# samanklesaria/traffic-env

Measured on AMD Instinct MI355X. Metric: vehicle_updates_per_sec, higher is better.
Workload: dtype f32; 1 GPU; cfg2: 4096 envs/GPU, 16x16 grid, L=400m, CAPACITY=66 (64 cars/road max), 48-car prefill, 1 spawn/entry road/8 ticks, 20-tick light cycle; settle_ticks=100, envs_per_gpu=4096, grid=16x16, cars_per_road_max=64, car_layout=transposed, parallelism=env-sharded x1

## Files before the change

### include/tfx.h

```cpp
#ifndef TFX_H
#define TFX_H

#include <stdint.h>

#ifdef __cplusplus
extern "C" {
#endif

#define TFX_ABI_VERSION 13
#define TFX_KP 2
#define TFX_MAX_ARCH 64

enum {
  TFX_OK = 0,
  TFX_EINVAL = -1,
  TFX_ESTATE = -2,
  TFX_EDEVICE = -3,
  TFX_ENOMEM = -4
};

enum {
  TFX_ACTION_BUFFER = 0,
  TFX_ACTION_BROADCAST = 1,
  TFX_ACTION_CYCLE = 2,
  TFX_ACTION_GREEDY = 3
};

enum {
  TFX_SPAWN_NONE = 0,
  TFX_SPAWN_COUNTS = 1,
  TFX_SPAWN_PERIODIC = 2
};

typedef struct tfx_config {
  int32_t m, n;
  int32_t capacity;
  int32_t n_envs;
  int32_t planes;
  float length;
  float rate;
  float car_v, car_l, car_a, car_delta, car_v0, car_b, car_T, car_s0;
  int32_t yellow_ticks;
  float thresh;
  float detect_dist;
  float overflow_penalty;
  float eps;
  int32_t learn_switch;
  int32_t validate;
  uint32_t entry_spec;
  int32_t env_id_offset;
  int32_t layout;
  int32_t n_archetypes;
  float arch[TFX_MAX_ARCH][8];
} tfx_config;

typedef struct tfx_buffers {
  float *xv;
  float *w;
  int32_t *leading;
  int32_t *lastcar;
  int32_t *obs;
  float *rewards;
  int32_t *waiting;
  uint8_t *passed_dst;
  int32_t *done_tick;
  float *trip_times;
  int32_t *n_trips;
  int32_t trip_cap;
} tfx_buffers;

typedef struct tfx_handle_s *tfx_handle;

int tfx_abi_version(void);
const char *tfx_last_error(void);

int tfx_create(const tfx_config *cfg, tfx_handle *out);
int tfx_destroy(tfx_handle h);
int tfx_dims(tfx_handle h, int32_t *I, int32_t *r, int32_t *R, int32_t *n_entry);
int tfx_tables(tfx_handle h, int32_t *dest, int32_t *phases, int32_t *nexts, int32_t *entrypoints);
int tfx_bind_buffers(tfx_handle h, const tfx_buffers *b);

int tfx_reset(tfx_handle h, const int32_t *phase_init, void *stream);
int tfx_reset_envs(tfx_handle h, const int32_t *phase_init, const uint8_t *mask, void *stream);
int tfx_refresh(tfx_handle h, void *stream);

int tfx_set_actions(tfx_handle h, int32_t mode, const int32_t *dev, int32_t period, int32_t per_tick);
int tfx_set_spawns(tfx_handle h, int32_t mode, const int32_t *dev, int32_t period, int32_t per_tick);
int tfx_set_poisson(tfx_handle h, double cars_per_tick, uint64_t seed, const uint32_t *cdf, int32_t n_cdf);
int tfx_set_regular(tfx_handle h, int32_t every, int32_t burst, uint64_t seed);
int tfx_set_spawn_archetypes(tfx_handle h, const uint8_t *dev, int32_t per_road, int32_t per_tick);

typedef struct tfx_demand {
  int32_t n_profiles, n_segments, seg_ticks, tick_offset, n_cdf;
  const uint32_t *count_cdf, *road_cdf;
  const int32_t *profile_of_env;
  uint64_t seed;
} tfx_demand;
int tfx_set_demand(tfx_handle h, const tfx_demand *dm);
int tfx_demand_counts(tfx_handle h, int32_t tick0, int32_t n_ticks, int32_t *out, void *stream);

int tfx_set_demand_mixed(tfx_handle h, const tfx_demand *dm, const uint32_t *row_cdf, int32_t n_rows);
int tfx_demand_rows(tfx_handle h, int32_t tick0, int32_t n_ticks, int32_t *counts, uint8_t *rows, void *stream);
int tfx_demand_rows_per_road(tfx_handle h, int32_t *per_road);

int tfx_step(tfx_handle h, int32_t n_ticks, void *stream);
int tfx_move_cars(tfx_handle h, void *stream);
int tfx_advance_finished_cars(tfx_handle h, void *stream);

int tfx_agent_step(tfx_handle h, int32_t n_ticks, int32_t remi, float *aobs, float *areward,
                   uint8_t *adone, void *stream);

typedef struct tfx_episode_buffers {
  float *ep_return;
  int32_t *ep_len;
  float *final_return;
  int32_t *final_len;
  uint8_t *truncated;
  int32_t *ep_index;
} tfx_episode_buffers;
int tfx_set_episodes(tfx_handle h, int32_t enabled, int32_t max_decisions, uint64_t seed, const tfx_episode_buffers *b);

int tfx_set_episode_pool(tfx_handle h, tfx_handle pool);

int tfx_remi(tfx_handle h, void *stream);
int tfx_cars_on_roads(tfx_handle h, int32_t *out, void *stream);
int tfx_done(tfx_handle h, uint8_t *out, int32_t since_tick, void *stream);

int tfx_get_tick(tfx_handle h, int32_t *tick);
int tfx_set_tick(tfx_handle h, int32_t tick);
int tfx_vehicle_updates(tfx_handle h, uint64_t *out, void *stream);
int tfx_reset_counters(tfx_handle h, void *stream);
int tfx_profile(tfx_handle h, int32_t max_ticks);
int tfx_profile_read(tfx_handle h, double *move_ms, double *advance_ms, int32_t *n_ticks);
int tfx_xv_pairs(tfx_handle h, int64_t *pairs);
int tfx_export_ring(tfx_handle h, float *ring_xv, float *ring_w, uint8_t *ring_a, void *stream);
int tfx_import_ring(tfx_handle h, const float *ring_xv, const float *ring_w, const uint8_t *ring_a, void *stream);

int tfx_fastdiv_status(tfx_handle h, int32_t *enabled, uint64_t *mismatches);
int tfx_launch_info(tfx_handle h, int32_t *grid, int32_t *block, int32_t *waves_per_road);
int tfx_fused_ticks(tfx_handle h, int64_t *ticks, int32_t *capable);
int tfx_pair_ticks(tfx_handle h, int64_t *ticks);
int tfx_tail_ticks(tfx_handle h, int64_t *ticks);
int tfx_slow_pairs(tfx_handle h, uint64_t *pairs, void *stream);
int tfx_split_ticks(tfx_handle h, int64_t *ticks);
const char *tfx_step_kernel(tfx_handle h);

int tfx_debug_fail_after(tfx_handle h, int32_t n_launches);

enum { TFX_CLONE_STREAM = 1, TFX_CLONE_EPISODE = 2 };
int tfx_clone_envs(tfx_handle dst, tfx_handle src, const int32_t *src_of_env, int32_t flags, void *stream);
int tfx_clone_skipped(tfx_handle h, uint64_t *skipped, void *stream);
typedef struct tfx_measure_buffers {
  int32_t *n_cars;
  int32_t *n_halted;
  int32_t *queue;
  float *speed_sum;
} tfx_measure_buffers;
enum { TFX_MEASURE_ACCUMULATE = 1 };
int tfx_road_measures(tfx_handle h, float halt_speed, float x_from, const tfx_measure_buffers *out, int32_t flags,
                      void *stream);
int tfx_measure_launch(tfx_handle h, int32_t *grid, int32_t *waves);
#define TFX_MAX_CELLS 32
typedef struct tfx_cell_buffers {
  int32_t *n_cars;
  float *speed_sum;
} tfx_cell_buffers;
enum { TFX_CELLS_ACCUMULATE = 1 };
int tfx_road_cells(tfx_handle h, const float *edges, int32_t n_cells, const tfx_cell_buffers *out, int32_t flags,
                   void *stream);
int tfx_cells_launch(tfx_handle h, int32_t n_cells, int32_t *grid, int32_t *waves);
#define TFX_FRAME_PX_MIN 8
#define TFX_FRAME_PX_MAX 256
enum { TFX_FRAMES_ROADS_ONLY = 1 };
int tfx_frame_size(tfx_handle h, int32_t px, int32_t *height, int32_t *width);
int tfx_frames(tfx_handle h, const int32_t *env_ids, int32_t n_frames, int32_t px, uint8_t *out, int32_t flags,
               void *stream);
int tfx_frames_launch(tfx_handle h, int32_t n_frames, int32_t px, int32_t *grid, int32_t *waves);
typedef struct tfx_age_buffers {
  int32_t *n_cars;
  int64_t *age_sum;
  int32_t *age_max;
} tfx_age_buffers;
enum { TFX_TRAVEL_ACCUMULATE = 1 };
int tfx_car_ages(tfx_handle h, const tfx_age_buffers *out, int32_t flags, void *stream);
int tfx_ages_launch(tfx_handle h, int32_t *grid, int32_t *waves);
typedef struct tfx_trip_stat_buffers {
  int32_t *count;
  int64_t *tick_sum;
  int32_t *tick_max;
  int32_t *lost;
  int32_t *hist;
} tfx_trip_stat_buffers;
int tfx_trip_stats(tfx_handle h, const int32_t *edges, int32_t n_bins, int32_t *cursor, const tfx_trip_stat_buffers *out,
                   int32_t flags, void *stream);
typedef struct tfx_follow_params {
  float x_from;
  float platoon_gap;
  float v_min;
  float ttc_crit;
} tfx_follow_params;
typedef struct tfx_follow_buffers {
  int32_t *n_cars;
  int32_t *n_pairs;
  int32_t *n_joined;
  int32_t *n_overlap;
  float *gap_sum;
  float *gap_min;
  int32_t *n_hw;
  float *hw_sum;
  int32_t *n_conflict;
  float *ttc_min;
  float *drac_max;
} tfx_follow_buffers;
enum { TFX_FOLLOW_ACCUMULATE = 1 };
int tfx_road_following(tfx_handle h, const tfx_follow_params *p, const tfx_follow_buffers *out, int32_t flags,
                       void *stream);
int tfx_follow_launch(tfx_handle h, int32_t *grid, int32_t *waves);
int tfx_debug_head_rows(tfx_handle h, uint8_t *out, void *stream);

typedef struct tfx_arrival_stream {
  uint32_t mt[624];
  int32_t pos;
  int32_t gap;
  int64_t tick;
} tfx_arrival_stream;
int tfx_arrivals_replay(tfx_arrival_stream *streams, int32_t n_streams, int32_t n_ticks, int32_t poisson,
                        double mean_gap, int32_t every, int32_t burst, int32_t n_choices,
                        const int32_t *column_of_choice, int32_t n_columns, int32_t *counts, int32_t *made);
int tfx_arrivals_replay_rows(tfx_arrival_stream *streams, int32_t n_streams, int32_t n_ticks, int32_t poisson,
                             double mean_gap, int32_t every, int32_t burst, int32_t n_choices,
                             const int32_t *column_of_choice, int32_t n_columns, int32_t *counts, int32_t *made,
                             int32_t n_archetypes, int32_t S, uint8_t *rows);

#ifdef __cplusplus
}
#endif
#endif
```

### traffic-env_amd/csrc/tfx_handle.hpp

```cpp
#pragma once
#include <hip/hip_runtime.h>

#include <cstdarg>
#include <cstdint>
#include <cstdio>
#include <cstdlib>
#include <cstring>
#include <string>
#include <vector>

#include "tfx.h"
#include "tfx_common.hpp"
#include "tfx_misc.hpp"
#include "tfx_demand.hpp"
#include "tfx_dev_layout.hpp"
#include "tfx_stream_layout.hpp"

using namespace tfx;

namespace {

thread_local std::string g_err;

int fail(int code, const char *fmt, ...) {
  char buf[512];
  va_list ap;
  va_start(ap, fmt);
  vsnprintf(buf, sizeof buf, fmt, ap);
  va_end(ap);
  g_err = buf;
  return code;
}

#define HIPCHK(expr)                                                                     \
  do {                                                                                   \
    hipError_t e_ = (expr);                                                              \
    if (e_ != hipSuccess) return fail(TFX_EDEVICE, "%s: %s", #expr, hipGetErrorString(e_)); \
  } while (0)

}

struct CapturedSeq {
  hipGraph_t graph = nullptr;
  hipGraphExec_t exec = nullptr;
  std::string key;
  long long fused = 0, pair = 0, tail = 0;
  const char *step_kernel = "";
};
enum { SEQ_AGENT = 0, SEQ_STEP = 1 };

enum StreamKind { STREAM_NONE, STREAM_POISSON, STREAM_REGULAR, STREAM_DEMAND };
struct ArrivalStream {
  StreamKind kind = STREAM_NONE;
  void *buf = nullptr;
  int *counts = nullptr;
  int rows = 1;
  int *gap = nullptr;
  unsigned *draws = nullptr, *sid = nullptr;
  unsigned *tables = nullptr;
  PoissonDev ps{};
  PoissonRows prow{};
  double rate = 0.0;
  DemandDev dm{};
  std::vector<uint32_t> count_cdf, road_cdf;
  DemandRows drow{};
  std::vector<uint32_t> row_cdf;
  bool mixed() const { return kind == STREAM_DEMAND && drow.row_cdf != nullptr; }
  bool drawn() const { return kind != STREAM_NONE; }
  bool upfront() const { return kind == STREAM_DEMAND; }
  bool stateful() const { return kind == STREAM_POISSON || kind == STREAM_REGULAR; }
};

struct tfx_handle_s {
  tfx_config cfg;
  Dev d;
  bool bound = false;
  int n_cu = 256;
  int wpr = 1;
  int grid_move = 0;
  int grid_tt[4] = {0, 0, 0, 0};
  int grid_edge = 0;
  int tt_segs = 0;
  int tt_seg = 1;
  int grid_adv = 0;
  int grid_tail = 0, grid_tail_half = 0;
  int tail_threads = 256, tail_threads_half = 128;
  int tail = 1;
  int split = 1;
  hipStream_t split_stream = nullptr;
  int split_prio = 0;
  hipEvent_t split_fork = nullptr, split_join = nullptr, split_stagger = nullptr;
  int split_half = -1;
  bool split_first = false;
  MiscWords *misc = nullptr;
  bool het = false;
  float *dev_arch = nullptr;
  long long split_ticks = 0;
  int pairs = 1;
  std::vector<int32_t> h_dest, h_phases, h_nexts, h_pred, h_entry, h_entry_idx, h_road_slot, h_slot_road;
  int *dev_tables = nullptr;
  int tiles_per_env = 0;
  int res_epb = 0;
  int res_lpr = 1;
  int res_threads = 0;
  size_t res_lds = 0;
  int res_min_ticks = 1;
  void *dev_scratch = nullptr;
  int32_t action_per_tick = 0, spawn_per_tick = 0;
  std::vector<hipEvent_t> ev;
  int ev_ticks = 0, ev_used = 0;
  std::vector<int> ev_weight;
  bool prof = false;
  long long fused_ticks = 0;
  long long pair_ticks = 0;
  long long tail_ticks = 0;
  const char *step_kernel = "";
  int move_variant = 0;
  int move_blocks_per_cu = 0;
  bool stagger = true;
  unsigned long long div_mismatches = 0;
  CapturedSeq captured[2];
  hipStream_t ag_stream = nullptr;
  unsigned long long input_gen = 0;
  bool use_graph = true;
  int fail_after = 0;
  ArrivalStream stream;
  bool greedy = false;
  int greedy_spacing = 3;
  int n_arch = 1;
  int *dev_greedy = nullptr;
  EpDev ep{};
  EpDev *dev_ep = nullptr;
  tfx_handle_s *pool = nullptr;
  int device = 0;
  int measure_grid = 0;
  int grid_cap = 0;
};

namespace {

void build_tables(tfx_handle_s *h) {
  const int m = h->cfg.m, n = h->cfg.n, v = m * n, r = 4 * v, R = r + 2 * m + 2 * n;
  h->h_dest.assign(R, -1);
  h->h_phases.assign(R, 0);
  h->h_nexts.assign(R, -1);
  h->h_pred.assign(R, -1);
  for (int dir = 0; dir < 4; ++dir)
    for (int row = 0; row < m; ++row)
      for (int col = 0; col < n; ++col) {
        const int li = row * n + col, e = dir * v + li;
        h->h_dest[e] = li;
        h->h_phases[e] = dir < 2 ? 1 : 0;
        int nx;
        switch (dir) {
          case 0: nx = col < n - 1 ? e + 1 : r + n + row; break;
          case 1: nx = col > 0 ? e - 1 : r + 2 * n + m + row; break;
          case 2: nx = row < m - 1 ? e + n : r + n + m + col; break;
          default: nx = row > 0 ? e - n : r + col; break;
        }
        h->h_nexts[e] = nx;
      }
  for (int e = 0; e < R; ++e)
    if (h->h_nexts[e] >= 0) h->h_pred[h->h_nexts[e]] = e;
  const uint32_t spec = h->cfg.entry_spec;
  h->h_entry.clear();
  if (!(spec & 1u)) for (int row = 0; row < m; ++row) h->h_entry.push_back(n * row);
  if (!((spec >> 1) & 1u)) for (int row = 1; row <= m; ++row) h->h_entry.push_back(v + n * row - 1);
  if (!((spec >> 2) & 1u)) for (int col = 0; col < n; ++col) h->h_entry.push_back(2 * v + col);
  if (!((spec >> 3) & 1u)) for (int col = 0; col < n; ++col) h->h_entry.push_back(3 * v + n * (m - 1) + col);
  h->h_entry_idx.assign(R, -1);
  for (size_t j = 0; j < h->h_entry.size(); ++j) h->h_entry_idx[h->h_entry[j]] = (int)j;
}

void build_slots(tfx_handle_s *h) {
  const int R = (int)h->h_nexts.size(), r = 4 * h->cfg.m * h->cfg.n;
  const char *kv = getenv("TFX_KINDS");
  std::vector<int> order;
  if (!(kv && atoi(kv) == 0)) {
    for (int e = 0; e < r; ++e) if (h->h_pred[e] >= 0) order.push_back(e);
    for (int e = 0; e < r; ++e) if (h->h_pred[e] < 0) order.push_back(e);
    for (int e = r; e < R; ++e) order.push_back(e);
  } else {
    for (int e = 0; e < R; ++e) order.push_back(e);
  }
  h->tiles_per_env = (R + 63) / 64;
  h->h_slot_road.assign((size_t)h->tiles_per_env * 64, -1);
  for (int s = 0; s < R; ++s) h->h_slot_road[s] = order[s];
  h->h_road_slot.assign(R, -1);
  for (size_t s = 0; s < h->h_slot_road.size(); ++s)
    if (h->h_slot_road[s] >= 0) h->h_road_slot[h->h_slot_road[s]] = (int)s;
}

bool inject_failure(tfx_handle h) {
  if (h->fail_after <= 0) return false;
  return --h->fail_after == 0;
}
#define TFX_INJECT(h)                                                                              \
  do {                                                                                             \
    if (inject_failure(h)) return fail(TFX_EDEVICE, "injected launch failure (tfx_debug_fail_after)"); \
  } while (0)

int check_handle(tfx_handle h, bool need_bound) {
  if (!h) return fail(TFX_EINVAL, "null handle");
  if (need_bound && !h->bound) return fail(TFX_ESTATE, "tfx_bind_buffers has not been called");
  return TFX_OK;
}

}
```

### traffic-env_amd/csrc/tfx_hip.hip

```cpp
#include <cmath>
#include <initializer_list>
#include <memory>
#include <new>

#include "tfx_cells.hpp"
#include "tfx_follow.hpp"
#include "tfx_frames.hpp"
#include "tfx_clone.hpp"
#include "tfx_measure.hpp"
#include "tfx_sequence.hpp"
#include "tfx_travel.hpp"

namespace {

template <class... T>
void key_put(std::string &key, const T &...v) {
  (key.append(reinterpret_cast<const char *>(&v), sizeof v), ...);
}
void key_put_arrays(std::string &key, const Dev &d) {
  for_each_env_array(d, [&key](const void *p, size_t, ArrayKind) { key_put(key, p); });
}

void stream_key(const ArrivalStream &a, std::string &key) {
  const PoissonDev &p = a.ps;
  const DemandDev &m = a.dm;
  key_put(key, a.kind, p.seed_lo, p.seed_hi, p.n_cdf, p.regular, p.every, p.burst, m.K, m.S, m.seg_ticks, m.tick_offset, m.n_cdf,
          m.seed_lo, m.seed_hi, m.profile, a.drow.n_rows, a.drow.S, a.buf);
}

std::string graph_key(tfx_handle h, int n_ticks, int remi, const void *aobs, const void *areward, const void *adone) {
  const Dev &d = h->d;
  static_assert(std::has_unique_object_representations_v<EpDev>, "the key takes the episode block byte for byte");
  std::string key;
  key.reserve(1024);
  key_put(key, h->input_gen, h->greedy, h->greedy_spacing, n_ticks, remi, aobs, areward, adone, d.action, d.action_mode,
          d.action_period, d.action_stride, d.spawn, d.spawn_mode, d.spawn_period, d.spawn_stride, h->pool);
  key_put_arrays(key, d);
  key_put(key, h->ep);
  if (const tfx_handle p = h->pool) {
    key_put_arrays(key, p->d);
    key_put(key, p->d.trip_cap, p->d.action_mode, p->d.spawn_mode);
  }
  stream_key(h->stream, key);
  return key;
}


template <class Body>
int run_captured(tfx_handle h, CapturedSeq &c, const std::string &key, hipStream_t st, Body body) {
  if (!c.exec || c.key != key) {
    if (c.exec) { (void)hipGraphExecDestroy(c.exec); c.exec = nullptr; }
    if (c.graph) { (void)hipGraphDestroy(c.graph); c.graph = nullptr; }
    if (!h->ag_stream) HIPCHK(hipStreamCreateWithFlags(&h->ag_stream, hipStreamNonBlocking));
    const long long fused0 = h->fused_ticks, pair0 = h->pair_ticks, tail0 = h->tail_ticks;
    HIPCHK(hipStreamBeginCapture(h->ag_stream, hipStreamCaptureModeThreadLocal));
    const int rc = body(h->ag_stream);
    hipGraph_t g = nullptr;
    const hipError_t ce = hipStreamEndCapture(h->ag_stream, &g);
    c.fused = h->fused_ticks - fused0;
    c.pair = h->pair_ticks - pair0;
    c.tail = h->tail_ticks - tail0;
    c.step_kernel = h->step_kernel;
    h->fused_ticks = fused0;
    h->pair_ticks = pair0;
    h->tail_ticks = tail0;
    if (rc != TFX_OK) { if (g) (void)hipGraphDestroy(g); return rc; }
    if (ce != hipSuccess) return fail(TFX_EDEVICE, "hipStreamEndCapture: %s", hipGetErrorString(ce));
    c.graph = g;
    HIPCHK(hipGraphInstantiate(&c.exec, g, nullptr, nullptr, 0));
    c.key = key;
  }
  HIPCHK(hipGraphLaunch(c.exec, st));
  h->fused_ticks += c.fused;
  h->pair_ticks += c.pair;
  h->tail_ticks += c.tail;
  h->step_kernel = c.step_kernel;
  return TFX_OK;
}

}

extern "C" int tfx_agent_step(tfx_handle h, int32_t n_ticks, int32_t remi, float *aobs, float *areward,
                              uint8_t *adone, void *stream) {
  if (int rc = check_handle(h, true)) return rc;
  if (n_ticks < 1) return fail(TFX_EINVAL, "n_ticks < 1");
  if (h->action_per_tick)
    return fail(TFX_EINVAL, "the fused agent step holds ONE action for all its ticks (bind the action buffer "
                            "with per_tick = 0)");
  if (h->stream.upfront() && n_ticks > h->stream.rows)
    return fail(TFX_EINVAL, "n_ticks = %d: a decision's arrivals are drawn up front and the demand's count buffer holds %d "
                            "rows at this batch size", n_ticks, h->stream.rows);
  hipStream_t st = (hipStream_t)stream;
  if (!res_usable(h, n_ticks)) {
    if (int rc = size_grids(h, true, n_ticks)) return rc;
  }
  const bool split = split_usable(h, n_ticks, true);
  if (split) {
    if (int rc = ensure_split(h, st)) return rc;
  }
  const bool capture = h->use_graph && !split;
  auto body = [&](hipStream_t s) { return agent_sequence(h, n_ticks, remi, aobs, areward, adone, s, split); };
  if (!capture) return body(st);
  return run_captured(h, h->captured[SEQ_AGENT], graph_key(h, n_ticks, remi, aobs, areward, adone), st, body);
}

namespace {

void drop_stream(tfx_handle h) {
  ArrivalStream &s = h->stream;
  if (!s.drawn()) return;
  Dev &d = h->d;
  if (d.spawn_arch && d.spawn_arch == s.prow.rows) {
    d.spawn_arch = nullptr;
    d.spawn_arch_S = 0;
    d.spawn_arch_stride = 0;
  }
  d.spawn = nullptr;
  d.spawn_stride = 0;
  d.spawn_mode = TFX_SPAWN_NONE;
  h->spawn_per_tick = 0;
  (void)hipFree(s.buf);
  s = ArrivalStream{};
}

struct HostTable { const uint32_t *words; size_t n; };
int stage_stream(tfx_handle h, StreamKind kind, uint64_t seed, std::initializer_list<HostTable> tables, ArrivalStream *out,
                 int demand_rows = 0) {
  const Dev &d = h->d;
  const bool demand = kind == STREAM_DEMAND;
  size_t n_tables = 0;
  for (const HostTable &t : tables) n_tables += t.n;
  const int S = kind == STREAM_POISSON && h->het ? d.C - 2 : (demand ? demand_rows : 0);
  const StreamLayout l = stream_layout(d.E, d.n_entry, n_tables, S, demand);
  ArrivalStream s;
  if (hipMalloc(&s.buf, l.bytes) != hipSuccess) {
    const hipError_t e = hipGetLastError();
    return demand ? fail(TFX_ENOMEM, "demand: hipMalloc(%zu bytes) failed", l.bytes)
                  : fail(TFX_EDEVICE, "hipMalloc(arrival stream, %zu bytes): %s", l.bytes, hipGetErrorString(e));
  }
  char *base = (char *)s.buf;
  s.kind = kind;
  s.rows = l.rows;
  s.counts = (int *)(base + l.counts);
  s.gap = (int *)(base + l.gap);
  s.draws = (unsigned *)(base + l.draws);
  s.sid = (unsigned *)(base + l.sid);
  s.tables = (unsigned *)(base + l.tables);
  std::vector<unsigned> ids((size_t)d.E);
  for (int e = 0; e < d.E; ++e) ids[(size_t)e] = (unsigned)(e + d.env_off);
  bool ok = hipMemset(s.buf, 0, l.bytes) == hipSuccess &&
            (kind != STREAM_POISSON || hipMemset(s.gap, 0xff, (size_t)d.E * 4) == hipSuccess) &&
            hipMemcpy(s.sid, ids.data(), ids.size() * 4, hipMemcpyHostToDevice) == hipSuccess;
  unsigned *to = s.tables;
  for (const HostTable &t : tables) {
    ok = ok && (t.n == 0 || hipMemcpy(to, t.words, t.n * 4, hipMemcpyHostToDevice) == hipSuccess);
    to += t.n;
  }
  if (!ok) {
    const hipError_t e = hipGetLastError();
    (void)hipFree(s.buf);
    return fail(TFX_EDEVICE, demand ? "demand: uploading the tables failed: %s" : "uploading the arrival stream failed: %s",
                hipGetErrorString(e));
  }
  if (demand) {
    s.dm.sid = s.sid;
    s.dm.seed_lo = (unsigned)seed;
    s.dm.seed_hi = (unsigned)(seed >> 32);
  } else {
    s.ps.counts = s.counts;
    s.ps.gap_left = s.gap;
    s.ps.draws = s.draws;
    s.ps.sid = s.sid;
    s.ps.seed_lo = (unsigned)seed;
    s.ps.seed_hi = (unsigned)(seed >> 32);
  }
  if (S > 0) {
    s.prow.seq = demand ? nullptr : (unsigned *)(base + l.seq);
    s.prow.rows = (uint8_t *)(base + l.arch);
    s.prow.S = S;
    s.prow.n_arch = h->n_arch;
  }
  *out = std::move(s);
  return TFX_OK;
}

void install_stream(tfx_handle h, ArrivalStream &&s) {
  Dev &d = h->d;
  ++h->input_gen;
  drop_stream(h);
  h->stream = std::move(s);
  const ArrivalStream &a = h->stream;
  d.spawn = a.counts;
  d.spawn_stride = a.upfront() ? (long)d.E * d.n_entry : 0;
  d.spawn_mode = TFX_SPAWN_COUNTS;
  h->spawn_per_tick = a.upfront() ? 1 : 0;
  d.spawn_arch = a.prow.rows;
  d.spawn_arch_S = a.prow.S;
  d.spawn_arch_stride = a.upfront() ? d.spawn_stride * a.prow.S : 0;
}

int bad_cdf_row(const uint32_t *row, int n) {
  for (int c = 1; c < n; ++c)
    if (row[c] < row[c - 1]) return c;
  return row[n - 1] != 0xFFFFFFFFu ? n : 0;
}

int set_demand(tfx_handle h, const tfx_demand *dm, bool mixed, const uint32_t *row_cdf, int32_t n_rows) {
  if (!dm) return fail(TFX_EINVAL, "demand: dm is null");
  if (!dm->count_cdf) return fail(TFX_EINVAL, "demand: count_cdf is null");
  if (!dm->road_cdf) return fail(TFX_EINVAL, "demand: road_cdf is null");
  if (mixed && !row_cdf) return fail(TFX_EINVAL, "demand: row_cdf is null");
  const int K = dm->n_profiles, S = dm->n_segments, n_cdf = dm->n_cdf;
  if (K < 1 || K > DEMAND_MAX_PROFILES) return fail(TFX_EINVAL, "demand: n_profiles %d is outside 1..%d", K, DEMAND_MAX_PROFILES);
  if (S < 1 || S > DEMAND_MAX_SEGMENTS) return fail(TFX_EINVAL, "demand: n_segments %d is outside 1..%d", S, DEMAND_MAX_SEGMENTS);
  if (dm->seg_ticks < 1) return fail(TFX_EINVAL, "demand: seg_ticks %d is below 1", dm->seg_ticks);
  if (n_cdf < 1 || n_cdf > DEMAND_MAX_CDF) return fail(TFX_EINVAL, "demand: n_cdf %d is outside 1..%d", n_cdf, DEMAND_MAX_CDF);
  if ((long long)S * dm->seg_ticks > 0x7fffffffLL)
    return fail(TFX_EINVAL, "demand: the period n_segments * seg_ticks = %lld does not fit an int32", (long long)S * dm->seg_ticks);
  for (int ks = 0; ks < K * S; ++ks)
    if (const int c = bad_cdf_row(dm->count_cdf + (size_t)ks * n_cdf, n_cdf))
      return fail(TFX_EINVAL, c < n_cdf ? "demand: count_cdf row (%d, %d) decreases at %d" : "demand: count_cdf row (%d, %d) does not end in 0xFFFFFFFF",
                  ks / S, ks % S, c);
  if (int rc = check_handle(h, false)) return rc;
  Dev &d = h->d;
  if (h->het && !mixed)
    return fail(TFX_EINVAL, "demand: heterogeneous handles (tfx_config.n_archetypes) are not supported - rule 4 draws no archetype rows: "
                            "tfx_set_demand_mixed draws them (rule 5)");
  if (mixed && !h->het)
    return fail(TFX_EINVAL, "demand: tfx_set_demand_mixed needs a heterogeneous handle (tfx_config.n_archetypes); this one has a "
                            "single archetype: tfx_set_demand");
  if (mixed && n_rows != h->n_arch)
    return fail(TFX_EINVAL, "demand: n_rows %d is not the handle's n_archetypes %d", n_rows, h->n_arch);
  if (d.n_entry < 1) return fail(TFX_EINVAL, "demand: no entry roads");
  if (d.n_entry > DEMAND_MAX_ENTRY) return fail(TFX_EINVAL, "demand: more than %d entry roads", DEMAND_MAX_ENTRY);
  const int ne = d.n_entry;
  for (int ks = 0; ks < K * S; ++ks)
    if (const int c = bad_cdf_row(dm->road_cdf + (size_t)ks * ne, ne))
      return fail(TFX_EINVAL, c < ne ? "demand: road_cdf row (%d, %d) decreases at %d" : "demand: road_cdf row (%d, %d) does not end in 0xFFFFFFFF",
                  ks / S, ks % S, c);
  for (int ks = 0; mixed && ks < K * S; ++ks)
    if (const int c = bad_cdf_row(row_cdf + (size_t)ks * n_rows, n_rows))
      return fail(TFX_EINVAL, c < n_rows ? "demand: row_cdf row (%d, %d) decreases at %d" : "demand: row_cdf row (%d, %d) does not end in 0xFFFFFFFF",
                  ks / S, ks % S, c);
  if (int rc = check_handle(h, true)) return rc;
  const size_t n_cc = (size_t)K * S * n_cdf, n_rc = (size_t)K * S * ne, n_rw = mixed ? (size_t)K * S * n_rows : 0;
  const int per_road = mixed ? (d.C - 2 < n_cdf - 1 ? d.C - 2 : n_cdf - 1) : 0;
  ArrivalStream s;
  if (int rc = stage_stream(h, STREAM_DEMAND, dm->seed, {{dm->count_cdf, n_cc}, {dm->road_cdf, n_rc}, {row_cdf, n_rw}}, &s, per_road))
    return rc;
  s.count_cdf.assign(dm->count_cdf, dm->count_cdf + n_cc);
  s.road_cdf.assign(dm->road_cdf, dm->road_cdf + n_rc);
  DemandDev &m = s.dm;
  m.count_cdf = s.tables;
  m.road_cdf = s.tables + n_cc;
  m.profile = dm->profile_of_env;
  m.K = K; m.S = S; m.seg_ticks = dm->seg_ticks; m.tick_offset = dm->tick_offset; m.n_cdf = n_cdf;
  if (mixed) {
    s.row_cdf.assign(row_cdf, row_cdf + n_rw);
    s.drow.row_cdf = s.tables + n_cc + n_rc;
    s.drow.n_rows = n_rows;
    s.drow.S = per_road;
  }
  install_stream(h, std::move(s));
  return TFX_OK;
}

template <class Body>
int for_stream_chunks(tfx_handle h, int n_ticks, hipStream_t st, Body body) {
  Dev &d = h->d;
  const ArrivalStream &s = h->stream;
  const int *const act0 = d.action;
  const long stride0 = d.spawn_stride, arch_stride0 = d.spawn_arch_stride;
  const bool rows = s.prow.rows && d.spawn_arch == s.prow.rows;
  int rc = TFX_OK;
  for (int done = 0; done < n_ticks && rc == TFX_OK; done += s.rows) {
    const int chunk = n_ticks - done < s.rows ? n_ticks - done : s.rows;
    rc = launch_stream(h, chunk, st);
    d.spawn_stride = (long)d.E * d.n_entry;
    if (rows) d.spawn_arch_stride = d.spawn_stride * s.prow.S;
    if (act0 && h->action_per_tick) d.action = act0 + (size_t)done * d.action_stride;
    if (rc == TFX_OK) rc = body(chunk);
    d.spawn_stride = stride0;
    d.spawn_arch_stride = arch_stride0;
    d.action = act0;
  }
  return rc;
}

int step_body(tfx_handle h, int n_ticks, hipStream_t st) {
  auto ticks = [&](int n) {
    const bool split = split_usable(h, n);
    if (split) {
      if (int rc = ensure_split(h, st)) return rc;
    }
    return run_ticks(h, n, st, false, split);
  };
  if (int rc = launch_greedy(h, st)) return rc;
  return h->stream.drawn() && n_ticks > 0 ? for_stream_chunks(h, n_ticks, st, ticks) : ticks(n_ticks);
}

struct ArchRows {
  int n = 1;
  bool het = false;
  float row[TFX_MAX_ARCH][8] = {};
};

int check_config(const tfx_config &cfg, ArchRows &ar) {
  if (cfg.m < 1 || cfg.n < 1) return fail(TFX_EINVAL, "grid must be at least 1x1");
  if (cfg.capacity < 3) return fail(TFX_EINVAL, "capacity must be >= 3 (slot 0 + fake leader + 1 car)");
  if (cfg.capacity - 2 > 256) return fail(TFX_EINVAL, "capacity-2 > 256 cars per road is not supported");
  if (cfg.n_envs < 1) return fail(TFX_EINVAL, "n_envs must be >= 1");
  if (cfg.planes != 2 && cfg.planes != 3) return fail(TFX_EINVAL, "planes must be 2 (x,v) or 3 (x,v,w)");
  if (cfg.validate && cfg.planes != 3) return fail(TFX_EINVAL, "validate mode needs planes = 3 (spawn tick w)");
  if (cfg.layout != 0 && cfg.layout != 1) return fail(TFX_EINVAL, "layout must be 0 (ring) or 1 (transposed)");
  ar.n = cfg.n_archetypes <= 1 ? 1 : cfg.n_archetypes;
  if (ar.n > TFX_MAX_ARCH) return fail(TFX_EINVAL, "at most %d archetype rows", TFX_MAX_ARCH);
  ar.het = ar.n > 1;
  for (int a = 0; a < ar.n; ++a) {
    const float single[8] = {cfg.car_v, cfg.car_l, cfg.car_a, cfg.car_delta, cfg.car_v0, cfg.car_b, cfg.car_T, cfg.car_s0};
    memcpy(ar.row[a], cfg.n_archetypes >= 1 ? cfg.arch[a] : single, sizeof single);
    const float delta = ar.row[a][3];
    if (!(delta > 0.0f) || !(delta <= 64.0f))
      return fail(TFX_EINVAL, "archetype %d: delta = %g - the exponent must be in (0, 64]", a, delta);
    if (delta != 4.0f) ar.het = true;
    if (!(ar.row[a][2] > 0.0f) || !(ar.row[a][5] > 0.0f) || !(ar.row[a][4] > 0.0f))
      return fail(TFX_EINVAL, "archetype %d: a, b and v0 must be > 0", a);
  }
  if (ar.het && (cfg.layout != 1 || cfg.planes != 3))
    return fail(TFX_EINVAL, "heterogeneous cars (several archetypes, or delta != 4) need layout = 1 and planes = 3");
  if (!(cfg.length > 0.0f) || !(cfg.rate > 0.0f)) return fail(TFX_EINVAL, "length and rate must be > 0");
  return TFX_OK;
}

int init_host(tfx_handle_s *h, const tfx_config &given, const ArchRows &ar) {
  h->cfg = given;
  h->het = ar.het;
  h->n_arch = ar.n;
  if (!ar.het && given.n_archetypes == 1) {
    h->cfg.car_v = ar.row[0][0]; h->cfg.car_l = ar.row[0][1]; h->cfg.car_a = ar.row[0][2];
    h->cfg.car_delta = ar.row[0][3]; h->cfg.car_v0 = ar.row[0][4]; h->cfg.car_b = ar.row[0][5];
    h->cfg.car_T = ar.row[0][6]; h->cfg.car_s0 = ar.row[0][7];
  }
  const tfx_config *cfg = &h->cfg;
  build_tables(h);
  build_slots(h);
  if (const char *mv = getenv("TFX_MOVE_VARIANT")) h->move_variant = atoi(mv);
  if (const char *gr = getenv("TFX_GRAPH")) h->use_graph = atoi(gr) != 0;
  if (const char *pv = getenv("TFX_PAIRS")) h->pairs = atoi(pv);
  if (const char *tv = getenv("TFX_TAIL")) h->tail = atoi(tv);
  if (const char *sv = getenv("TFX_SPLIT")) h->split = atoi(sv);
  if (const char *gv = getenv("TFX_TT_SEG")) h->tt_seg = atoi(gv);
  if (const char *gv = getenv("TFX_TT_SEGS")) h->tt_segs = atoi(gv);
  if (const char *gv = getenv("TFX_MEASURE_GRID")) h->measure_grid = atoi(gv);
  if (const char *gv = getenv("TFX_GRID_CAP")) h->grid_cap = atoi(gv) > 0 ? atoi(gv) : 0;
  if (const char *pc = getenv("TFX_MOVE_BLOCKS_PER_CU")) h->move_blocks_per_cu = atoi(pc);
  if (const char *sv = getenv("TFX_STAGGER")) h->stagger = atoi(sv) != 0;
  int dev = 0;
  hipDeviceProp_t prop;
  if (hipGetDevice(&dev) == hipSuccess) h->device = dev;
  if (hipGetDeviceProperties(&prop, dev) == hipSuccess)
    h->n_cu = prop.multiProcessorCount > 0 ? prop.multiProcessorCount : 256;

  Dev &d = h->d;
  memset(&d, 0, sizeof d);
  d.I = cfg->m * cfg->n;
  d.r = 4 * d.I;
  d.R = d.r + 2 * cfg->m + 2 * cfg->n;
  d.C = cfg->capacity;
  d.E = cfg->n_envs;
  d.n_entry = (int)h->h_entry.size();
  d.obs_len = 2 * d.r + 2 * d.I;
  d.yellow = cfg->yellow_ticks;
  d.learn_switch = cfg->learn_switch;
  d.validate = cfg->validate;
  d.env_off = cfg->env_id_offset;
  d.layout = cfg->layout;
  d.length = cfg->length;
  d.rate = cfg->rate;
  d.car_v = cfg->car_v; d.car_l = cfg->car_l; d.car_a = cfg->car_a; d.car_v0 = cfg->car_v0;
  d.car_b = cfg->car_b; d.car_T = cfg->car_T; d.car_s0 = cfg->car_s0;
  d.risk_a = cfg->car_a;
  if (ar.het)
    for (int a = 0; a < ar.n; ++a) d.risk_a = a == 0 ? ar.row[0][2] : fmaxf(d.risk_a, ar.row[a][2]);
  d.two_sab = 2.0f * sqrtf(cfg->car_a * cfg->car_b);
  d.eps = cfg->eps;
  d.r_two_sab = 1.0f / d.two_sab;
  d.r_v0 = 1.0f / cfg->car_v0;
  d.thresh = cfg->thresh;
  d.near_end = cfg->length - cfg->detect_dist;
  d.ovf_pen = cfg->overflow_penalty;
  if ((long)d.E * d.R > 0x7fffffffL / 4) return fail(TFX_EINVAL, "E*R too large");
  d.G = h->tiles_per_env;
  d.trows = d.C - 2;
  d.het = ar.het ? 1 : 0;
  const int cars = d.C - 2;
  h->wpr = cars <= 64 ? 1 : (cars <= 128 ? 2 : 4);
  d.action_mode = TFX_ACTION_CYCLE;
  d.action_period = 20;
  d.spawn_mode = TFX_SPAWN_NONE;
  d.spawn_period = 8;
  return TFX_OK;
}

int init_device(tfx_handle_s *h, const ArchRows &ar) {
  Dev &d = h->d;
  const size_t R = (size_t)d.R;
  const size_t n_slots = h->h_slot_road.size();
  if (hipMalloc((void **)&h->dev_tables, (4 * R + n_slots) * sizeof(int)) != hipSuccess)
    return fail(TFX_ENOMEM, "hipMalloc(tables) failed");
  if (hipMemcpy(h->dev_tables, h->h_nexts.data(), R * sizeof(int), hipMemcpyHostToDevice) != hipSuccess ||
      hipMemcpy(h->dev_tables + R, h->h_pred.data(), R * sizeof(int), hipMemcpyHostToDevice) != hipSuccess ||
      hipMemcpy(h->dev_tables + 2 * R, h->h_entry_idx.data(), R * sizeof(int), hipMemcpyHostToDevice) != hipSuccess ||
      hipMemcpy(h->dev_tables + 3 * R, h->h_road_slot.data(), R * sizeof(int), hipMemcpyHostToDevice) != hipSuccess ||
      hipMemcpy(h->dev_tables + 4 * R, h->h_slot_road.data(), n_slots * sizeof(int), hipMemcpyHostToDevice) != hipSuccess)
    return fail(TFX_EDEVICE, "uploading the road tables failed");
  d.nexts = h->dev_tables;
  d.pred = h->dev_tables + R;
  d.entry_idx = h->dev_tables + 2 * R;
  d.road_slot = h->dev_tables + 3 * R;
  d.slot_road = h->dev_tables + 4 * R;

  const size_t bytes = carve_arena(d, h->ep, h->dev_ep, h->misc, h->cfg.planes, nullptr);
  if (hipMalloc(&h->dev_scratch, bytes) != hipSuccess) return fail(TFX_ENOMEM, "hipMalloc(scratch, %zu bytes) failed", bytes);
  if (hipMemset(h->dev_scratch, 0, bytes) != hipSuccess) return fail(TFX_EDEVICE, "clearing the scratch failed");
  carve_arena(d, h->ep, h->dev_ep, h->misc, h->cfg.planes, (char *)h->dev_scratch);
  if (ar.het) {
    float tab[TFX_MAX_ARCH][ARCH_W] = {};
    for (int a = 0; a < ar.n; ++a) {
      const float *r = ar.row[a];
      tab[a][AR_L] = r[1]; tab[a][AR_A] = r[2]; tab[a][AR_V0] = r[4]; tab[a][AR_T] = r[6]; tab[a][AR_S0] = r[7];
      tab[a][AR_2SAB] = 2.0f * sqrtf(r[2] * r[5]);
      tab[a][AR_DELTA] = r[3]; tab[a][AR_V] = r[0];
    }
    if (hipMalloc((void **)&h->dev_arch, sizeof tab) != hipSuccess ||
        hipMemcpy(h->dev_arch, tab, sizeof tab, hipMemcpyHostToDevice) != hipSuccess)
      return fail(TFX_ENOMEM, "uploading the archetype table failed");
    d.arch_tab = h->dev_arch;
  }
  d.fastdiv = 0;
  {
    const char *fd = getenv("TFX_FASTDIV");
    if (!fd || atoi(fd) != 0) {
      unsigned long long *bad = &h->misc->selftest;
      hipLaunchKernelGGL(k_div_selftest, dim3(h->n_cu * 8), dim3(256), 0, 0, d.two_sab, d.r_two_sab,
                         TFX_FASTDIV_A_LO, TFX_FASTDIV_A_HI, bad);
      hipLaunchKernelGGL(k_div_selftest, dim3(h->n_cu * 8), dim3(256), 0, 0, h->cfg.car_v0, d.r_v0,
                         TFX_FASTDIV_V_LO, TFX_FASTDIV_V_HI, bad);
      unsigned long long nbad = 1;
      if (hipMemcpy(&nbad, bad, sizeof nbad, hipMemcpyDeviceToHost) == hipSuccess && nbad == 0) d.fastdiv = 1;
      (void)hipMemset(bad, 0, sizeof nbad);
      h->div_mismatches = nbad;
    }
  }
  {
    unsigned *bad = reinterpret_cast<unsigned *>(&h->misc->selftest);
    hipLaunchKernelGGL(k_max_selftest, dim3(1), dim3(1), 0, 0, bad, 0.0f, -0.0f);
    unsigned nbad = 1;
    if (hipMemcpy(&nbad, bad, sizeof nbad, hipMemcpyDeviceToHost) == hipSuccess && nbad == 0) d.fastmax = 1;
    (void)hipMemset(bad, 0, 8);
  }
  return TFX_OK;
}

}

extern "C" {

int tfx_abi_version(void) { return TFX_ABI_VERSION; }
const char *tfx_last_error(void) { return g_err.c_str(); }

int tfx_create(const tfx_config *cfg, tfx_handle *out) {
  if (!cfg || !out) return fail(TFX_EINVAL, "null argument");
  ArchRows ar;
  if (int rc = check_config(*cfg, ar)) return rc;
  int ndev = 0;
  HIPCHK(hipGetDeviceCount(&ndev));
  if (ndev < 1) return fail(TFX_EDEVICE, "no HIP device");
  std::unique_ptr<tfx_handle_s, int (*)(tfx_handle)> h(new (std::nothrow) tfx_handle_s(), tfx_destroy);
  if (!h) return fail(TFX_ENOMEM, "out of host memory");
  if (int rc = init_host(h.get(), *cfg, ar)) return rc;
  if (int rc = init_device(h.get(), ar)) return rc;
  *out = h.release();
  return TFX_OK;
}

int tfx_destroy(tfx_handle h) {
  if (!h) return TFX_OK;
  for (hipEvent_t e : h->ev) (void)hipEventDestroy(e);
  for (CapturedSeq &c : h->captured) {
    if (c.exec) (void)hipGraphExecDestroy(c.exec);
    if (c.graph) (void)hipGraphDestroy(c.graph);
  }
  if (h->ag_stream) (void)hipStreamDestroy(h->ag_stream);
  if (h->split_stream) {
    (void)hipStreamSynchronize(h->split_stream);
    (void)hipStreamDestroy(h->split_stream);
    (void)hipEventDestroy(h->split_fork);
    (void)hipEventDestroy(h->split_join);
    (void)hipEventDestroy(h->split_stagger);
  }
  drop_stream(h);
  if (h->dev_greedy) (void)hipFree(h->dev_greedy);
  if (h->dev_tables) (void)hipFree(h->dev_tables);
  if (h->dev_scratch) (void)hipFree(h->dev_scratch);
  if (h->dev_arch) (void)hipFree(h->dev_arch);
  delete h;
  return TFX_OK;
}

int tfx_dims(tfx_handle h, int32_t *I, int32_t *r, int32_t *R, int32_t *n_entry) {
  if (int rc = check_handle(h, false)) return rc;
  if (I) *I = h->d.I;
  if (r) *r = h->d.r;
  if (R) *R = h->d.R;
  if (n_entry) *n_entry = h->d.n_entry;
  return TFX_OK;
}

int tfx_tables(tfx_handle h, int32_t *dest, int32_t *phases, int32_t *nexts, int32_t *entrypoints) {
  if (int rc = check_handle(h, false)) return rc;
  const size_t R = (size_t)h->d.R;
  if (dest) memcpy(dest, h->h_dest.data(), R * sizeof(int32_t));
  if (phases) memcpy(phases, h->h_phases.data(), R * sizeof(int32_t));
  if (nexts) memcpy(nexts, h->h_nexts.data(), R * sizeof(int32_t));
  if (entrypoints) memcpy(entrypoints, h->h_entry.data(), h->h_entry.size() * sizeof(int32_t));
  return TFX_OK;
}

int tfx_bind_buffers(tfx_handle h, const tfx_buffers *b) {
  if (int rc = check_handle(h, false)) return rc;
  if (!b) return fail(TFX_EINVAL, "null buffers");
  if (!b->xv || !b->leading || !b->lastcar || !b->obs || !b->rewards || !b->waiting ||
      !b->passed_dst || !b->done_tick)
    return fail(TFX_EINVAL, "xv, leading, lastcar, obs, rewards, waiting, passed_dst and done_tick are required");
  if (h->cfg.planes == 3 && !b->w) return fail(TFX_EINVAL, "planes = 3 needs the w buffer");
  if (((uintptr_t)b->xv & 15u) != 0) return fail(TFX_EINVAL, "xv must be 16-byte aligned");
  if (h->cfg.validate && (!b->n_trips || (b->trip_times && b->trip_cap < 1)))
    return fail(TFX_EINVAL, "validate mode needs n_trips (and trip_cap >= 1 with trip_times)");
  Dev &d = h->d;
  d.xv = reinterpret_cast<float2 *>(b->xv); d.w = b->w;
  d.leading = b->leading; d.lastcar = b->lastcar; d.obs = b->obs;
  d.lights = env_lights(d); d.lights_stride = d.obs_len;
  d.rewards = b->rewards; d.waiting = b->waiting; d.passed_dst = b->passed_dst;
  d.done_tick = b->done_tick; d.trip_times = b->trip_times; d.n_trips = b->n_trips;
  d.trip_cap = b->trip_cap;
  h->bound = true;
  ++h->input_gen;
  return d.w ? res_configure<true>(h) : res_configure<false>(h);
}

int tfx_reset(tfx_handle h, const int32_t *phase_init, void *stream) {
  if (int rc = check_handle(h, true)) return rc;
  if (!phase_init) return fail(TFX_EINVAL, "phase_init is required");
  hipStream_t st = (hipStream_t)stream;
  HIPCHK(hipMemsetAsync(h->d.tickA, 0, sizeof(int), st));
  HIPCHK(hipMemsetAsync(h->d.tickB, 0, sizeof(int), st));
  hipLaunchKernelGGL(k_reset, dim3(grid_for(h, (long)h->d.E * h->d.R)), dim3(256), 0, st, h->d, phase_init,
                     (const uint8_t *)nullptr, h->ep);
  HIPCHK(hipGetLastError());
  return TFX_OK;
}

int tfx_reset_envs(tfx_handle h, const int32_t *phase_init, const uint8_t *mask, void *stream) {
  if (int rc = check_handle(h, true)) return rc;
  if (!phase_init || !mask) return fail(TFX_EINVAL, "phase_init and mask are required");
  hipLaunchKernelGGL(k_reset, dim3(grid_for(h, (long)h->d.E * h->d.R)), dim3(256), 0, (hipStream_t)stream,
                     h->d, phase_init, mask, h->ep);
  HIPCHK(hipGetLastError());
  return TFX_OK;
}

int tfx_set_episodes(tfx_handle h, int32_t enabled, int32_t max_decisions, uint64_t seed, const tfx_episode_buffers *b) {
  if (enabled) {
    if (max_decisions < 0) return fail(TFX_EINVAL, "max_decisions must be >= 0 (0: no time limit)");
    if (!b) return fail(TFX_EINVAL, "null episode buffers");
    if (!b->ep_return || !b->ep_len || !b->final_return || !b->final_len || !b->truncated || !b->ep_index)
      return fail(TFX_EINVAL, "ep_return, ep_len, final_return, final_len, truncated and ep_index are required");
  }
  if (int rc = check_handle(h, true)) return rc;
  EpDev &ep = h->ep;
  HIPCHK(hipDeviceSynchronize());
  HIPCHK(hipMemset(ep.mark, 0, 2 * (size_t)h->d.E));
  ++h->input_gen;
  ep.on = enabled ? 1 : 0;
  ep.max = enabled ? max_decisions : 0;
  ep.seed_lo = enabled ? (unsigned)seed : 0u;
  ep.seed_hi = enabled ? (unsigned)(seed >> 32) : 0u;
  ep.ep_return = enabled ? b->ep_return : nullptr;
  ep.ep_len = enabled ? b->ep_len : nullptr;
  ep.final_return = enabled ? b->final_return : nullptr;
  ep.final_len = enabled ? b->final_len : nullptr;
  ep.trunc = enabled ? b->truncated : nullptr;
  ep.ep_index = enabled ? b->ep_index : nullptr;
  HIPCHK(hipMemcpy(h->dev_ep, &ep, sizeof ep, hipMemcpyHostToDevice));
  HIPCHK(hipDeviceSynchronize());
  return TFX_OK;
}

int tfx_refresh(tfx_handle h, void *stream) {
  if (int rc = check_handle(h, true)) return rc;
  hipLaunchKernelGGL(k_refresh, dim3(grid_for(h, (long)h->d.E * h->d.R)), dim3(256), 0,
                     (hipStream_t)stream, h->d);
  HIPCHK(hipGetLastError());
  return TFX_OK;
}

int tfx_set_actions(tfx_handle h, int32_t mode, const int32_t *dev, int32_t period, int32_t per_tick) {
  if (int rc = check_handle(h, false)) return rc;
  Dev &d = h->d;
  ++h->input_gen;
  h->greedy = false;
  d.greedy_spacing = 0;
  d.greedy_act = nullptr;
  if (mode == TFX_ACTION_GREEDY) {
    if (period < 1) return fail(TFX_EINVAL, "greedy spacing must be >= 1");
    if (!h->dev_greedy) {
      HIPCHK(hipMalloc((void **)&h->dev_greedy, (size_t)d.E * d.I * sizeof(int)));
      HIPCHK(hipMemset(h->dev_greedy, 0, (size_t)d.E * d.I * sizeof(int)));
    }
    h->greedy = true;
    h->greedy_spacing = period;
    d.greedy_spacing = period;
    d.greedy_act = h->dev_greedy;
    d.action = h->dev_greedy;
    d.action_stride = 0;
    d.action_mode = TFX_ACTION_BUFFER;
    h->action_per_tick = 0;
    return TFX_OK;
  }
  if (mode == TFX_ACTION_CYCLE) {
    if (period < 1) return fail(TFX_EINVAL, "cycle period must be >= 1");
    d.action_period = period;
  } else if (mode == TFX_ACTION_BUFFER || mode == TFX_ACTION_BROADCAST) {
    if (!dev) return fail(TFX_EINVAL, "action buffer is null");
    d.action = dev;
    d.action_stride = per_tick ? (mode == TFX_ACTION_BUFFER ? (long)d.E * d.I : (long)d.I) : 0;
  } else {
    return fail(TFX_EINVAL, "unknown action mode %d", mode);
  }
  d.action_mode = mode;
  h->action_per_tick = per_tick;
  return TFX_OK;
}

int tfx_set_spawns(tfx_handle h, int32_t mode, const int32_t *dev, int32_t period, int32_t per_tick) {
  if (int rc = check_handle(h, false)) return rc;
  Dev &d = h->d;
  ++h->input_gen;
  drop_stream(h);
  if (mode == TFX_SPAWN_PERIODIC) {
    if (period < 1) return fail(TFX_EINVAL, "spawn period must be >= 1");
    d.spawn_period = period;
  } else if (mode == TFX_SPAWN_COUNTS) {
    if (!dev) return fail(TFX_EINVAL, "spawn buffer is null");
    d.spawn = dev;
    d.spawn_stride = per_tick ? (long)d.E * d.n_entry : 0;
  } else if (mode != TFX_SPAWN_NONE) {
    return fail(TFX_EINVAL, "unknown spawn mode %d", mode);
  }
  d.spawn_mode = mode;
  h->spawn_per_tick = per_tick;
  return TFX_OK;
}

int tfx_set_spawn_archetypes(tfx_handle h, const uint8_t *dev, int32_t per_road, int32_t per_tick) {
  if (int rc = check_handle(h, false)) return rc;
  if (!h->het) return fail(TFX_ESTATE, "the handle has a single archetype");
  if (dev && per_road < 1) return fail(TFX_EINVAL, "per_road must be >= 1");
  Dev &d = h->d;
  ++h->input_gen;
  d.spawn_arch = dev;
  d.spawn_arch_S = dev ? per_road : 0;
  d.spawn_arch_stride = (dev && per_tick) ? (long)d.E * d.n_entry * per_road : 0;
  return TFX_OK;
}

int tfx_set_poisson(tfx_handle h, double cars_per_tick, uint64_t seed, const uint32_t *cdf, int32_t n_cdf) {
  if (int rc = check_handle(h, false)) return rc;
  if (!(cars_per_tick > 0.0)) return fail(TFX_EINVAL, "cars_per_tick must be > 0");
  if (!cdf || n_cdf < 1 || n_cdf > 65536) return fail(TFX_EINVAL, "gap table missing or too long");
  Dev &d = h->d;
  if (d.n_entry < 1) return fail(TFX_EINVAL, "no entry roads");
  ArrivalStream s;
  if (int rc = stage_stream(h, STREAM_POISSON, seed, {{cdf, (size_t)n_cdf}}, &s)) return rc;
  s.ps.cdf = s.tables;
  s.ps.n_cdf = n_cdf;
  s.rate = cars_per_tick;
  install_stream(h, std::move(s));
  return TFX_OK;
}

int tfx_set_regular(tfx_handle h, int32_t every, int32_t burst, uint64_t seed) {
  if (int rc = check_handle(h, false)) return rc;
  if (every < 0 || burst < 1) return fail(TFX_EINVAL, "every must be >= 0 and burst >= 1");
  Dev &d = h->d;
  if (d.n_entry < 1) return fail(TFX_EINVAL, "no entry roads");
  ArrivalStream s;
  if (int rc = stage_stream(h, STREAM_REGULAR, seed, {}, &s)) return rc;
  s.ps.regular = 1;
  s.ps.every = every;
  s.ps.burst = burst;
  install_stream(h, std::move(s));
  return TFX_OK;
}

int tfx_set_demand(tfx_handle h, const tfx_demand *dm) { return set_demand(h, dm, false, nullptr, 0); }

int tfx_set_demand_mixed(tfx_handle h, const tfx_demand *dm, const uint32_t *row_cdf, int32_t n_rows) {
  return set_demand(h, dm, true, row_cdf, n_rows);
}

int tfx_demand_counts(tfx_handle h, int32_t tick0, int32_t n_ticks, int32_t *out, void *stream) {
  if (!out) return fail(TFX_EINVAL, "demand: out is null");
  if (n_ticks < 0) return fail(TFX_EINVAL, "demand: n_ticks %d is negative", n_ticks);
  if (int rc = check_handle(h, true)) return rc;
  if (!h->stream.upfront()) return fail(TFX_ESTATE, "demand: tfx_set_demand has not been called (or another spawn rule replaced it)");
  if (n_ticks == 0) return TFX_OK;
  return launch_demand(h, 0, tick0, n_ticks, out, nullptr, (hipStream_t)stream);
}

int tfx_demand_rows(tfx_handle h, int32_t tick0, int32_t n_ticks, int32_t *counts, uint8_t *rows, void *stream) {
  if (!counts) return fail(TFX_EINVAL, "demand: counts is null");
  if (!rows) return fail(TFX_EINVAL, "demand: rows is null");
  if (n_ticks < 0) return fail(TFX_EINVAL, "demand: n_ticks %d is negative", n_ticks);
  if (int rc = check_handle(h, true)) return rc;
  if (!h->stream.mixed())
    return fail(TFX_ESTATE, "demand: tfx_set_demand_mixed has not been called (or another spawn rule replaced it)");
  if (n_ticks == 0) return TFX_OK;
  return launch_demand(h, 0, tick0, n_ticks, counts, h->stream.drow.S > 0 ? rows : nullptr, (hipStream_t)stream);
}

int tfx_demand_rows_per_road(tfx_handle h, int32_t *per_road) {
  if (!per_road) return fail(TFX_EINVAL, "demand: per_road is null");
  if (int rc = check_handle(h, true)) return rc;
  if (!h->stream.mixed())
    return fail(TFX_ESTATE, "demand: tfx_set_demand_mixed has not been called (or another spawn rule replaced it)");
  *per_road = h->stream.drow.S;
  return TFX_OK;
}

int tfx_step(tfx_handle h, int32_t n_ticks, void *stream) {
  if (int rc = check_handle(h, true)) return rc;
  if (n_ticks < 0) return fail(TFX_EINVAL, "n_ticks < 0");
  hipStream_t st = (hipStream_t)stream;
  if (n_ticks > 0 && res_usable(h, n_ticks)) {
    auto fused = [&](int n) {
      TickTimer timer(h);
      if (int rc = timer.begin(st)) return rc;
      if (int rc = launch_res(h, n, st)) return rc;
      h->fused_ticks += n;
      if (int rc = timer.mid(st)) return rc;
      return timer.end(st, n);
    };
    return h->stream.upfront() ? for_stream_chunks(h, n_ticks, st, fused) : fused(n_ticks);
  }
  if (int rc = size_grids(h, false, n_ticks)) return rc;
  const Dev &d = h->d;
  const bool capture = h->use_graph && !h->prof && n_ticks >= 4 && d.layout == 1 &&
                       (long)d.E * d.G <= (long)h->n_cu * 24 && !split_usable(h, n_ticks);
  auto body = [&](hipStream_t s) { return step_body(h, n_ticks, s); };
  if (!capture) return body(st);
  return run_captured(h, h->captured[SEQ_STEP], graph_key(h, n_ticks, -1, nullptr, nullptr, nullptr), st, body);
}

int tfx_move_cars(tfx_handle h, void *stream) {
  if (int rc = check_handle(h, true)) return rc;
  if (int rc = size_grids(h, false, 1)) return rc;
  if (int rc = launch_greedy(h, (hipStream_t)stream)) return rc;
  if (int rc = h->stream.upfront() ? launch_stream(h, 1, (hipStream_t)stream) : launch_inputs(h, (hipStream_t)stream)) return rc;
  return (pairs_usable(h) && !single_tick_ts(h)) ? launch_move_tt(h, false, false, 0, (hipStream_t)stream) : launch_move(h, 0, (hipStream_t)stream);
}

int tfx_advance_finished_cars(tfx_handle h, void *stream) {
  if (int rc = check_handle(h, true)) return rc;
  if (int rc = size_grids(h, false, 1)) return rc;
  return launch_advance(h, 0, (hipStream_t)stream);
}

int tfx_remi(tfx_handle h, void *stream) {
  if (int rc = check_handle(h, true)) return rc;
  hipLaunchKernelGGL(k_remi, dim3(grid_for(h, (long)h->d.E * h->d.I)), dim3(256), 0,
                     (hipStream_t)stream, h->d);
  HIPCHK(hipGetLastError());
  return TFX_OK;
}

int tfx_cars_on_roads(tfx_handle h, int32_t *out, void *stream) {
  if (int rc = check_handle(h, true)) return rc;
  if (!out) return fail(TFX_EINVAL, "out is null");
  hipLaunchKernelGGL(k_cars_on_roads, dim3(grid_for(h, (long)h->d.E * h->d.R)), dim3(256), 0,
                     (hipStream_t)stream, h->d, out);
  HIPCHK(hipGetLastError());
  return TFX_OK;
}

int tfx_done(tfx_handle h, uint8_t *out, int32_t since_tick, void *stream) {
  if (int rc = check_handle(h, true)) return rc;
  if (!out) return fail(TFX_EINVAL, "out is null");
  hipLaunchKernelGGL(k_done, dim3(grid_for(h, h->d.E)), dim3(256), 0, (hipStream_t)stream, h->d,
                     out, since_tick);
  HIPCHK(hipGetLastError());
  return TFX_OK;
}

int tfx_get_tick(tfx_handle h, int32_t *tick) {
  if (int rc = check_handle(h, false)) return rc;
  if (!tick) return fail(TFX_EINVAL, "tick is null");
  HIPCHK(hipDeviceSynchronize());
  HIPCHK(hipMemcpy(tick, h->d.tickA, sizeof(int), hipMemcpyDeviceToHost));
  return TFX_OK;
}

int tfx_set_tick(tfx_handle h, int32_t tick) {
  if (int rc = check_handle(h, false)) return rc;
  HIPCHK(hipDeviceSynchronize());
  HIPCHK(hipMemcpy(h->d.tickA, &tick, sizeof(int), hipMemcpyHostToDevice));
  HIPCHK(hipMemcpy(h->d.tickB, &tick, sizeof(int), hipMemcpyHostToDevice));
  HIPCHK(hipMemset(h->d.env_flag, 0, (size_t)h->d.E * sizeof(int)));
  if (h->bound) HIPCHK(hipMemset(h->d.done_tick, 0, (size_t)h->d.E * sizeof(int)));
  return TFX_OK;
}

int tfx_vehicle_updates(tfx_handle h, uint64_t *out, void *stream) {
  if (int rc = check_handle(h, false)) return rc;
  if (!out) return fail(TFX_EINVAL, "out is null");
  HIPCHK(hipStreamSynchronize((hipStream_t)stream));
  std::vector<unsigned long long> slots((size_t)VEH_SLOTS * VEH_STRIDE);
  HIPCHK(hipMemcpy(slots.data(), h->d.veh, slots.size() * sizeof(unsigned long long), hipMemcpyDeviceToHost));
  unsigned long long v = 0;
  for (int i = 0; i < VEH_SLOTS; ++i) v += slots[(size_t)i * VEH_STRIDE];
  *out = (uint64_t)v;
  return TFX_OK;
}

int tfx_reset_counters(tfx_handle h, void *stream) {
  if (int rc = check_handle(h, false)) return rc;
  HIPCHK(hipMemsetAsync(h->d.veh, 0, (size_t)VEH_SLOTS * VEH_STRIDE * sizeof(unsigned long long), (hipStream_t)stream));
  return TFX_OK;
}

int tfx_profile(tfx_handle h, int32_t max_ticks) {
  if (int rc = check_handle(h, false)) return rc;
  for (hipEvent_t e : h->ev) (void)hipEventDestroy(e);
  h->ev.clear();
  h->ev_ticks = 0;
  h->ev_used = 0;
  h->prof = max_ticks > 0;
  if (!h->prof) return TFX_OK;
  h->ev.resize((size_t)max_ticks * 3);
  h->ev_weight.assign((size_t)max_ticks, 1);
  for (hipEvent_t &e : h->ev) HIPCHK(hipEventCreate(&e));
  h->ev_ticks = max_ticks;
  return TFX_OK;
}

int tfx_profile_read(tfx_handle h, double *move_ms, double *advance_ms, int32_t *n_ticks) {
  if (int rc = check_handle(h, false)) return rc;
  double mv = 0.0, ad = 0.0;
  int ticks = 0;
  for (int i = 0; i < h->ev_used; ++i) {
    float a = 0.f, b = 0.f;
    HIPCHK(hipEventSynchronize(h->ev[(size_t)i * 3 + 2]));
    HIPCHK(hipEventElapsedTime(&a, h->ev[(size_t)i * 3], h->ev[(size_t)i * 3 + 1]));
    HIPCHK(hipEventElapsedTime(&b, h->ev[(size_t)i * 3 + 1], h->ev[(size_t)i * 3 + 2]));
    mv += a;
    ad += b;
    ticks += h->ev_weight[i];
  }
  if (move_ms) *move_ms = mv;
  if (advance_ms) *advance_ms = ad;
  if (n_ticks) *n_ticks = ticks;
  h->ev_used = 0;
  return TFX_OK;
}

int tfx_xv_pairs(tfx_handle h, int64_t *pairs) {
  if (int rc = check_handle(h, false)) return rc;
  if (!pairs) return fail(TFX_EINVAL, "pairs is null");
  *pairs = (int64_t)h->d.E * (int64_t)env_car_pairs(h->d);
  return TFX_OK;
}

int tfx_export_ring(tfx_handle h, float *ring_xv, float *ring_w, uint8_t *ring_a, void *stream) {
  if (int rc = check_handle(h, true)) return rc;
  if (h->d.layout != 1) return fail(TFX_ESTATE, "the handle already uses the ring layout");
  if (!ring_xv) return fail(TFX_EINVAL, "ring_xv is null");
  hipLaunchKernelGGL(k_export_ring, dim3(grid_for(h, (long)h->d.E * h->d.R)), dim3(256), 0,
                     (hipStream_t)stream, h->d, reinterpret_cast<float2 *>(ring_xv), ring_w, ring_a);
  HIPCHK(hipGetLastError());
  return TFX_OK;
}

int tfx_import_ring(tfx_handle h, const float *ring_xv, const float *ring_w, const uint8_t *ring_a, void *stream) {
  if (int rc = check_handle(h, true)) return rc;
  if (h->d.layout != 1) return fail(TFX_ESTATE, "the handle already uses the ring layout");
  if (!ring_xv) return fail(TFX_EINVAL, "ring_xv is null");
  hipLaunchKernelGGL(k_import_ring, dim3(grid_for(h, (long)h->d.E * h->d.R)), dim3(256), 0,
                     (hipStream_t)stream, h->d, reinterpret_cast<const float2 *>(ring_xv), ring_w, ring_a);
  HIPCHK(hipGetLastError());
  return TFX_OK;
}

int tfx_fastdiv_status(tfx_handle h, int32_t *enabled, uint64_t *mismatches) {
  if (int rc = check_handle(h, false)) return rc;
  if (enabled) *enabled = h->d.fastdiv;
  if (mismatches) *mismatches = h->div_mismatches;
  return TFX_OK;
}

int tfx_fused_ticks(tfx_handle h, int64_t *ticks, int32_t *capable) {
  if (int rc = check_handle(h, false)) return rc;
  if (ticks) *ticks = h->fused_ticks;
  if (capable) *capable = h->res_epb > 0 ? 1 : 0;
  return TFX_OK;
}

int tfx_pair_ticks(tfx_handle h, int64_t *ticks) {
  if (int rc = check_handle(h, false)) return rc;
  if (ticks) *ticks = h->pair_ticks;
  return TFX_OK;
}

int tfx_tail_ticks(tfx_handle h, int64_t *ticks) {
  if (int rc = check_handle(h, false)) return rc;
  if (ticks) *ticks = h->tail_ticks;
  return TFX_OK;
}

int tfx_slow_pairs(tfx_handle h, uint64_t *pairs, void *stream) {
  if (int rc = check_handle(h, false)) return rc;
  if (!pairs) return fail(TFX_EINVAL, "pairs is null");
  HIPCHK(hipStreamSynchronize((hipStream_t)stream));
  unsigned long long v = 0;
  HIPCHK(hipMemcpy(&v, h->d.slow_pairs, sizeof v, hipMemcpyDeviceToHost));
  *pairs = (uint64_t)v;
  return TFX_OK;
}

int tfx_split_ticks(tfx_handle h, int64_t *ticks) {
  if (int rc = check_handle(h, false)) return rc;
  if (ticks) *ticks = h->split_ticks;
  return TFX_OK;
}

const char *tfx_step_kernel(tfx_handle h) { return h ? h->step_kernel : ""; }

}

namespace {

int same_world(tfx_handle dst, tfx_handle src, const char *what) {
  const tfx_config &a = dst->cfg, &b = src->cfg;
  if (dst->device != src->device)
    return fail(TFX_EINVAL, "%s: the handles live on different devices (device %d / %d)", what, dst->device, src->device);
#define TFX_SAME(field, fmt)                                                                                         \
  if (a.field != b.field) return fail(TFX_EINVAL, "%s: the handles differ in " #field " (" fmt " / " fmt ")", what, a.field, b.field)
  TFX_SAME(m, "%d"); TFX_SAME(n, "%d"); TFX_SAME(capacity, "%d"); TFX_SAME(planes, "%d"); TFX_SAME(layout, "%d");
  TFX_SAME(length, "%g"); TFX_SAME(rate, "%g"); TFX_SAME(validate, "%d"); TFX_SAME(learn_switch, "%d");
  TFX_SAME(entry_spec, "%u");
  TFX_SAME(yellow_ticks, "%d"); TFX_SAME(thresh, "%g"); TFX_SAME(detect_dist, "%g"); TFX_SAME(overflow_penalty, "%g");
  TFX_SAME(eps, "%g");
#undef TFX_SAME
  if (dst->het != src->het || dst->n_arch != src->n_arch)
    return fail(TFX_EINVAL, "%s: the handles differ in n_archetypes (%d / %d rows)", what, dst->n_arch, src->n_arch);
  const bool table = a.n_archetypes >= 1;
  if (table != (b.n_archetypes >= 1) ||
      (table ? memcmp(a.arch, b.arch, (size_t)dst->n_arch * sizeof a.arch[0]) != 0
             : (a.car_v != b.car_v || a.car_l != b.car_l || a.car_a != b.car_a || a.car_delta != b.car_delta ||
                a.car_v0 != b.car_v0 || a.car_b != b.car_b || a.car_T != b.car_T || a.car_s0 != b.car_s0)))
    return fail(TFX_EINVAL, "%s: the handles differ in the archetype table (arch)", what);
  if (dst->h_slot_road != src->h_slot_road)
    return fail(TFX_EINVAL, "%s: the handles differ in the kinds ordering of their storage slots (TFX_KINDS)", what);
  return TFX_OK;
}

int streams_compatible(tfx_handle dst, tfx_handle src) {
  const ArrivalStream &a = dst->stream, &b = src->stream;
  if (a.upfront() != b.upfront())
    return fail(TFX_EINVAL, "clone: the handles differ in the stream kind (demand profiles in one handle only)");
  if (a.upfront()) {
    const DemandDev &p = a.dm, &q = b.dm;
    if (p.seed_lo != q.seed_lo || p.seed_hi != q.seed_hi) return fail(TFX_EINVAL, "clone: the handles differ in the demand seed");
    if (p.K != q.K || p.S != q.S || p.seg_ticks != q.seg_ticks || p.n_cdf != q.n_cdf)
      return fail(TFX_EINVAL, "clone: the handles differ in the demand sizes (n_profiles, n_segments, seg_ticks, n_cdf)");
    if (p.tick_offset != q.tick_offset) return fail(TFX_EINVAL, "clone: the handles differ in the demand tick_offset");
    if (a.count_cdf != b.count_cdf || a.road_cdf != b.road_cdf || a.row_cdf != b.row_cdf)
      return fail(TFX_EINVAL, "clone: the handles differ in the demand tables (count_cdf / road_cdf / row_cdf)");
    return TFX_OK;
  }
  if (!a.drawn() || !b.drawn())
    return fail(TFX_EINVAL, "clone: TFX_CLONE_STREAM needs an on-device arrival stream (tfx_set_poisson / tfx_set_regular / "
                            "tfx_set_demand) in both handles");
  const PoissonDev &p = a.ps, &q = b.ps;
  if (p.regular != q.regular) return fail(TFX_EINVAL, "clone: the handles differ in the stream kind (poisson / regular)");
  if (p.seed_lo != q.seed_lo || p.seed_hi != q.seed_hi) return fail(TFX_EINVAL, "clone: the handles differ in the stream seed");
  if (p.regular ? (p.every != q.every) : (a.rate != b.rate || p.n_cdf != q.n_cdf))
    return fail(TFX_EINVAL, "clone: the handles differ in the stream rate");
  if (p.burst != q.burst) return fail(TFX_EINVAL, "clone: the handles differ in the stream burst");
  return TFX_OK;
}

}

extern "C" {

int tfx_clone_envs(tfx_handle dst, tfx_handle src, const int32_t *src_of_env, int32_t flags, void *stream) {
  if (flags & ~(TFX_CLONE_STREAM | TFX_CLONE_EPISODE)) return fail(TFX_EINVAL, "unknown clone flags 0x%x", flags);
  if (!src_of_env) return fail(TFX_EINVAL, "src_of_env is null");
  if (int rc = check_handle(dst, true)) return rc;
  if (int rc = check_handle(src, true)) return rc;
  if (dst != src) {
    if (int rc = same_world(dst, src, "clone")) return rc;
  }
  CloneOpt o{};
  o.same = dst == src ? 1 : 0;
  o.skipped = &dst->misc->clone_skipped;
  if (flags & TFX_CLONE_STREAM) {
    if (int rc = streams_compatible(dst, src)) return rc;
    const ArrivalStream &p = dst->stream, &q = src->stream;
    o.stream = 1;
    o.d_gap = p.gap; o.s_gap = q.gap;
    o.d_draws = p.draws; o.s_draws = q.draws;
    o.d_sid = p.sid; o.s_sid = q.sid;
    o.d_seq = p.prow.seq; o.s_seq = q.prow.seq;
  }
  if (flags & TFX_CLONE_EPISODE) {
    if (dst->ep.on != src->ep.on)
      return fail(TFX_EINVAL, "clone: TFX_CLONE_EPISODE with episodes on in one handle only (tfx_set_episodes)");
    if (dst->ep.on) {
      o.episode = 1;
      o.d_ep = dst->ep;
      o.s_ep = src->ep;
    }
  }
  if (dst->d.greedy_act && src->d.greedy_act) {
    o.d_greedy = dst->d.greedy_act;
    o.s_greedy = src->d.greedy_act;
  }
  TFX_INJECT(dst);
  hipLaunchKernelGGL(k_clone<false>, dim3((unsigned)tile_grid(dst)), dim3(256), 0, (hipStream_t)stream, dst->d, src->d,
                     (const int *)src_of_env, o);
  HIPCHK(hipGetLastError());
  return TFX_OK;
}

int tfx_set_episode_pool(tfx_handle h, tfx_handle pool) {
  if (int rc = check_handle(h, false)) return rc;
  if (pool == h) return fail(TFX_EINVAL, "episode pool: a handle cannot be its own pool");
  if (int rc = check_handle(h, true)) return rc;
  if (pool) {
    if (int rc = check_handle(pool, true)) return rc;
    if (int rc = same_world(h, pool, "episode pool")) return rc;
  }
  h->pool = pool;
  ++h->input_gen;
  return TFX_OK;
}

int tfx_clone_skipped(tfx_handle h, uint64_t *skipped, void *stream) {
  if (int rc = check_handle(h, false)) return rc;
  if (!skipped) return fail(TFX_EINVAL, "skipped is null");
  unsigned long long v = 0;
  HIPCHK(hipMemcpyAsync(&v, &h->misc->clone_skipped, sizeof v, hipMemcpyDeviceToHost, (hipStream_t)stream));
  HIPCHK(hipMemsetAsync(&h->misc->clone_skipped, 0, sizeof v, (hipStream_t)stream));
  HIPCHK(hipStreamSynchronize((hipStream_t)stream));
  *skipped = (uint64_t)v;
  return TFX_OK;
}

int tfx_road_measures(tfx_handle h, float halt_speed, float x_from, const tfx_measure_buffers *out, int32_t flags,
                      void *stream) {
  if (!out) return fail(TFX_EINVAL, "out is null");
  if (int rc = check_handle(h, false)) return rc;
  if (!out->n_cars && !out->n_halted && !out->queue && !out->speed_sum)
    return fail(TFX_EINVAL, "measures: every output pointer is null");
  if (flags & ~TFX_MEASURE_ACCUMULATE) return fail(TFX_EINVAL, "unknown measure flags 0x%x", flags);
  if (std::isnan(halt_speed) || std::isnan(x_from)) return fail(TFX_EINVAL, "measures: halt_speed / x_from is NaN");
  if (int rc = check_handle(h, true)) return rc;
  MeasureOut o{};
  o.n_cars = out->n_cars;
  o.n_halted = out->n_halted;
  o.queue = out->queue;
  o.speed_sum = out->speed_sum;
  o.accumulate = (flags & TFX_MEASURE_ACCUMULATE) ? 1 : 0;
  return launch_query(k_measure, tile_grid(h, true), stream, h->d, halt_speed, x_from, o);
}

int tfx_measure_launch(tfx_handle h, int32_t *grid, int32_t *waves) {
  if (int rc = check_handle(h, false)) return rc;
  return report_launch(tile_grid(h, true), grid, waves);
}

int tfx_road_following(tfx_handle h, const tfx_follow_params *p, const tfx_follow_buffers *out, int32_t flags,
                       void *stream) {
  if (!p) return fail(TFX_EINVAL, "following: p is null");
  if (!out) return fail(TFX_EINVAL, "following: out is null");
  if (int rc = check_handle(h, false)) return rc;
  if (!out->n_cars && !out->n_pairs && !out->n_joined && !out->n_overlap && !out->gap_sum && !out->gap_min && !out->n_hw &&
      !out->hw_sum && !out->n_conflict && !out->ttc_min && !out->drac_max)
    return fail(TFX_EINVAL, "following: every output pointer is null");
  if (flags & ~TFX_FOLLOW_ACCUMULATE) return fail(TFX_EINVAL, "unknown following flags 0x%x", flags);
  if (std::isnan(p->x_from) || std::isnan(p->platoon_gap) || std::isnan(p->v_min) || std::isnan(p->ttc_crit))
    return fail(TFX_EINVAL, "following: x_from / platoon_gap / v_min / ttc_crit is NaN");
  if (!(p->v_min > 0.0f)) return fail(TFX_EINVAL, "following: v_min %g is not above 0", (double)p->v_min);
  if (int rc = check_handle(h, true)) return rc;
  FollowOut o{};
  o.n_cars = out->n_cars;
  o.n_pairs = out->n_pairs;
  o.n_joined = out->n_joined;
  o.n_overlap = out->n_overlap;
  o.gap_sum = out->gap_sum;
  o.gap_min = out->gap_min;
  o.n_hw = out->n_hw;
  o.hw_sum = out->hw_sum;
  o.n_conflict = out->n_conflict;
  o.ttc_min = out->ttc_min;
  o.drac_max = out->drac_max;
  o.accumulate = (flags & TFX_FOLLOW_ACCUMULATE) ? 1 : 0;
  return launch_query(k_follow, tile_grid(h, true), stream, h->d, *p, o);
}

int tfx_follow_launch(tfx_handle h, int32_t *grid, int32_t *waves) {
  if (int rc = check_handle(h, false)) return rc;
  return report_launch(tile_grid(h, true), grid, waves);
}

int tfx_car_ages(tfx_handle h, const tfx_age_buffers *out, int32_t flags, void *stream) {
  if (!out) return fail(TFX_EINVAL, "ages: out is null");
  if (int rc = check_handle(h, false)) return rc;
  if (!out->n_cars && !out->age_sum && !out->age_max) return fail(TFX_EINVAL, "ages: every output pointer is null");
  if (flags & ~TFX_TRAVEL_ACCUMULATE) return fail(TFX_EINVAL, "unknown travel flags 0x%x", flags);
  if (int rc = check_handle(h, true)) return rc;
  if (!h->d.w) return fail(TFX_ESTATE, "ages: the handle carries no side plane (planes == 2): spawn ticks are not kept");
  AgeOut o{};
  o.n_cars = out->n_cars;
  o.age_sum = reinterpret_cast<long long *>(out->age_sum);
  o.age_max = out->age_max;
  o.accumulate = (flags & TFX_TRAVEL_ACCUMULATE) ? 1 : 0;
  return launch_query(k_ages, tile_grid(h, true), stream, h->d, o);
}

int tfx_ages_launch(tfx_handle h, int32_t *grid, int32_t *waves) {
  if (int rc = check_handle(h, false)) return rc;
  return report_launch(tile_grid(h, true), grid, waves);
}

int tfx_trip_stats(tfx_handle h, const int32_t *edges, int32_t n_bins, int32_t *cursor, const tfx_trip_stat_buffers *out,
                   int32_t flags, void *stream) {
  if (!out) return fail(TFX_EINVAL, "trips: out is null");
  if (int rc = check_handle(h, false)) return rc;
  if (!out->count && !out->tick_sum && !out->tick_max && !out->lost && !out->hist)
    return fail(TFX_EINVAL, "trips: every output pointer is null");
  if (flags & ~TFX_TRAVEL_ACCUMULATE) return fail(TFX_EINVAL, "unknown travel flags 0x%x", flags);
  if (n_bins < 0 || n_bins > TRIP_BINS || (out->hist && n_bins < 1))
    return fail(TFX_EINVAL, "trips: n_bins %d is outside 1..%d", n_bins, TRIP_BINS);
  TripEdges ed{};
  if (out->hist) {
    if (!edges) return fail(TFX_EINVAL, "trips: hist is given but edges is null");
    for (int k = 0; k < n_bins; ++k)
      if (edges[k] > edges[k + 1])
        return fail(TFX_EINVAL, "trips: edges decrease at %d (%d, %d)", k, edges[k], edges[k + 1]);
    for (int k = 0; k <= TRIP_BINS; ++k) ed.e[k] = edges[k <= n_bins ? k : n_bins];
  }
  if (int rc = check_handle(h, true)) return rc;
  if (!h->d.validate || !h->d.trip_times || !h->d.n_trips)
    return fail(TFX_ESTATE, "trips: the handle is not in validate mode with trip_times and n_trips bound: no trip log is kept");
  TripOut o{};
  o.count = out->count;
  o.tick_sum = reinterpret_cast<long long *>(out->tick_sum);
  o.tick_max = out->tick_max;
  o.lost = out->lost;
  o.hist = out->hist;
  o.accumulate = (flags & TFX_TRAVEL_ACCUMULATE) ? 1 : 0;
  return launch_query(k_trips, item_grid(h, h->d.E), stream, h->d, ed, out->hist ? n_bins : 0, cursor, o);
}

int tfx_road_cells(tfx_handle h, const float *edges, int32_t n_cells, const tfx_cell_buffers *out, int32_t flags,
                   void *stream) {
  if (!edges) return fail(TFX_EINVAL, "cells: edges is null");
  if (!out) return fail(TFX_EINVAL, "cells: out is null");
  if (!out->n_cars && !out->speed_sum) return fail(TFX_EINVAL, "cells: every output pointer is null");
  if (n_cells < 1 || n_cells > TFX_MAX_CELLS)
    return fail(TFX_EINVAL, "cells: n_cells %d is outside 1..%d", n_cells, TFX_MAX_CELLS);
  if (flags & ~TFX_CELLS_ACCUMULATE) return fail(TFX_EINVAL, "unknown cell flags 0x%x", flags);
  for (int k = 0; k <= n_cells; ++k)
    if (std::isnan(edges[k])) return fail(TFX_EINVAL, "cells: edge %d is NaN", k);
  for (int k = 0; k < n_cells; ++k)
    if (!(edges[k] < edges[k + 1]))
      return fail(TFX_EINVAL, "cells: edges are not strictly ascending at %d (%g, %g)", k, edges[k], edges[k + 1]);
  if (int rc = check_handle(h, true)) return rc;
  CellEdges ed;
  ed.lo = edges[0];
  ed.hi = edges[n_cells];
  for (int k = 0; k < TFX_MAX_CELLS; ++k) ed.inner[k] = (k >= 1 && k < n_cells) ? edges[k] : INFINITY;
  CellOut o{};
  o.n_cars = out->n_cars;
  o.speed_sum = out->speed_sum;
  o.accumulate = (flags & TFX_CELLS_ACCUMULATE) ? 1 : 0;
  const int B = n_cells;
  return launch_query(B <= 8 ? k_cells<8> : B <= 16 ? k_cells<16> : k_cells<32>, tile_grid(h, true), stream, h->d, ed, B, o);
}

int tfx_cells_launch(tfx_handle h, int32_t n_cells, int32_t *grid, int32_t *waves) {
  if (int rc = check_handle(h, false)) return rc;
  if (n_cells < 1 || n_cells > TFX_MAX_CELLS)
    return fail(TFX_EINVAL, "cells: n_cells %d is outside 1..%d", n_cells, TFX_MAX_CELLS);
  return report_launch(tile_grid(h, true), grid, waves);
}

static int frame_px_ok(int32_t px) {
  if (px < TFX_FRAME_PX_MIN || px > TFX_FRAME_PX_MAX)
    return fail(TFX_EINVAL, "frames: px %d is outside %d..%d", px, TFX_FRAME_PX_MIN, TFX_FRAME_PX_MAX);
  return TFX_OK;
}

int tfx_frame_size(tfx_handle h, int32_t px, int32_t *height, int32_t *width) {
  if (int rc = frame_px_ok(px)) return rc;
  if (int rc = check_handle(h, false)) return rc;
  if (height) *height = (h->cfg.m + 1) * px + 1;
  if (width) *width = (h->cfg.n + 1) * px + 1;
  return TFX_OK;
}

int tfx_frames(tfx_handle h, const int32_t *env_ids, int32_t n_frames, int32_t px, uint8_t *out, int32_t flags,
               void *stream) {
  if (!out) return fail(TFX_EINVAL, "frames: out is null");
  if (n_frames < 1) return fail(TFX_EINVAL, "frames: n_frames %d is less than 1", n_frames);
  if (int rc = frame_px_ok(px)) return rc;
  if (flags & ~TFX_FRAMES_ROADS_ONLY) return fail(TFX_EINVAL, "unknown frame flags 0x%x", flags);
  if (int rc = check_handle(h, false)) return rc;
  if (!env_ids && n_frames > h->d.E)
    return fail(TFX_EINVAL, "frames: n_frames %d is more than the handle's %d envs and env_ids is null", n_frames, h->d.E);
  const long long W = (long long)(h->cfg.n + 1) * px + 1, H = (long long)(h->cfg.m + 1) * px + 1;
  if (W * H > 0x7fffffffll) return fail(TFX_EINVAL, "frames: a frame of %lld x %lld pixels is too large", H, W);
  if (int rc = check_handle(h, true)) return rc;
  FrameArgs f{};
  f.env_ids = env_ids;
  f.out = reinterpret_cast<unsigned *>(out);
  f.n_frames = n_frames;
  f.roads_only = (flags & TFX_FRAMES_ROADS_ONLY) ? 1 : 0;
  f.m = h->cfg.m;
  f.n = h->cfg.n;
  f.S = px;
  f.W = (int)W;
  f.H = (int)H;
  f.k = (float)(px - 3) / h->cfg.length;
  if (!(flags & TFX_FRAMES_ROADS_ONLY))
    HIPCHK(hipMemsetAsync(out, 0xFF, (size_t)n_frames * (size_t)(W * H) * 4, (hipStream_t)stream));
  return launch_query(k_frames, tile_grid(h, true, n_frames), stream, h->d, f);
}

int tfx_frames_launch(tfx_handle h, int32_t n_frames, int32_t px, int32_t *grid, int32_t *waves) {
  if (n_frames < 1) return fail(TFX_EINVAL, "frames: n_frames %d is less than 1", n_frames);
  if (int rc = frame_px_ok(px)) return rc;
  if (int rc = check_handle(h, false)) return rc;
  return report_launch(tile_grid(h, true, n_frames), grid, waves);
}

int tfx_debug_head_rows(tfx_handle h, uint8_t *out, void *stream) {
  if (int rc = check_handle(h, true)) return rc;
  if (!out) return fail(TFX_EINVAL, "out is null");
  const size_t n = (size_t)h->d.E * h->d.R;
  HIPCHK(hipStreamSynchronize((hipStream_t)stream));
  if (h->d.layout != 1) {
    memset(out, 0, n);
    return TFX_OK;
  }
  HIPCHK(hipMemcpy(out, h->d.hb, n, hipMemcpyDeviceToHost));
  return TFX_OK;
}

int tfx_debug_fail_after(tfx_handle h, int32_t n_launches) {
  if (int rc = check_handle(h, false)) return rc;
  h->fail_after = n_launches > 0 ? n_launches : 0;
  return TFX_OK;
}

int tfx_launch_info(tfx_handle h, int32_t *grid, int32_t *block, int32_t *waves_per_road) {
  if (int rc = check_handle(h, false)) return rc;
  if (h->grid_move == 0) return fail(TFX_ESTATE, "no move kernel has been launched yet");
  if (grid) *grid = h->grid_move;
  if (block) *block = 256;
  if (waves_per_road) *waves_per_road = h->wpr;
  return TFX_OK;
}

}

#include "tfx_arrivals.cpp"
```

### traffic-env_amd/csrc/tfx_misc.hpp

```cpp
#pragma once
#include "tfx_common.hpp"
#include "tfx_move_t.hpp"

namespace tfx {

__device__ __forceinline__ void reset_road(const Dev &d, const int env, const int e, const long id, const int phase) {
  if (d.layout == 0) {
    d.xv[(size_t)id * d.C + 1] = make_float2(INFINITY, 0.0f);
    if (d.w) d.w[(size_t)id * d.C + 1] = 0.0f;
  } else {
    d.leadx[id] = INFINITY;
    d.hb[id] = 0;
  }
  d.leading[id] = 1;
  d.lastcar[id] = 1;
  d.tailx[id] = 0.0f;
  d.rec[id] = make_int4(0, 0, 0, 0);
  int *ob = d.obs + (size_t)env * d.obs_len;
  if (e < d.r) {
    ob[e] = 0;
    d.waiting[(size_t)env * d.r + e] = 0;
  }
  if (e < d.I) {
    ob[2 * d.r + e] = phase;
    ob[2 * d.r + d.I + e] = 0;
    d.passed_dst[(size_t)env * d.I + e] = 0;
  }
  if (e == 0) {
    d.done_tick[env] = 0;
    d.env_flag[env] = 0;
    if (d.n_trips) d.n_trips[env] = 0;
  }
}

__global__ void k_reset(const Dev d, const int *phase_init, const uint8_t *mask, const EpDev ep) {
  const long total = (long)d.E * d.R;
  for (long id = (long)blockIdx.x * blockDim.x + threadIdx.x; id < total;
       id += (long)gridDim.x * blockDim.x) {
    const int env = (int)(id / d.R);
    const int e = (int)(id - (long)env * d.R);
    if (mask && !mask[env]) continue;
    reset_road(d, env, e, id, e < d.I ? phase_init[(size_t)env * d.I + e] : 0);
    if (ep.on) {
      if (e < d.I) ep.ep_return[(size_t)env * d.I + e] = 0.0f;
      if (e == 0) {
        ep.ep_len[env] = 0;
        ep.mark[env] = 0;
      }
    }
  }
}

__global__ void k_refresh(const Dev d) {
  const long total = (long)d.E * d.R;
  for (long id = (long)blockIdx.x * blockDim.x + threadIdx.x; id < total;
       id += (long)gridDim.x * blockDim.x)
  {
    if (d.layout == 0) {
      d.tailx[id] = d.xv[(size_t)id * d.C + d.lastcar[id]].x;
    } else {
      const int n = ring_count(d.leading[id], d.lastcar[id], d.C);
      const int hb = d.hb[id];
      d.tailx[id] = (n > 0) ? d.xv[tpos(d, (int)id, n - 1 + hb)].x : 0.0f;
      if (d.het) d.taila[id] = (n > 0) ? side_arch(d.w[tpos(d, (int)id, n - 1 + hb)]) : 0;
    }
  }
}

__global__ void k_export_ring(const Dev d, float2 *ring, float *ringw, uint8_t *ringa) {
  const long total = (long)d.E * d.R;
  for (long id = (long)blockIdx.x * blockDim.x + threadIdx.x; id < total;
       id += (long)gridDim.x * blockDim.x) {
    const int ld = d.leading[id];
    const int n = ring_count(ld, d.lastcar[id], d.C);
    float2 *row = ring + (size_t)id * d.C;
    const int hb = d.layout == 1 ? d.hb[id] : 0;
    int slot = ld;
    for (int k = 0; k < n; ++k) {
      slot = wrap1(slot + 1, d.C);
      row[slot] = d.xv[tpos(d, (int)id, k + hb)];
      if (d.w && (ringw || ringa)) {
        const float sw = d.w[tpos(d, (int)id, k + hb)];
        if (ringw) ringw[(size_t)id * d.C + slot] = side_tick(d, sw);
        if (ringa) ringa[(size_t)id * d.C + slot] = d.het ? (uint8_t)side_arch(sw) : 0;
      }
    }
    row[ld].x = d.leadx[id];
  }
}

__global__ void k_import_ring(const Dev d, const float2 *ring, const float *ringw, const uint8_t *ringa) {
  const long total = (long)d.E * d.R;
  for (long id = (long)blockIdx.x * blockDim.x + threadIdx.x; id < total;
       id += (long)gridDim.x * blockDim.x) {
    const int ld = d.leading[id];
    const int n = ring_count(ld, d.lastcar[id], d.C);
    const float2 *row = ring + (size_t)id * d.C;
    int slot = ld;
    for (int k = 0; k < n; ++k) {
      slot = wrap1(slot + 1, d.C);
      d.xv[tpos(d, (int)id, k)] = row[slot];
      if (d.w && (ringw || (d.het && ringa))) {
        const float tk = ringw ? ringw[(size_t)id * d.C + slot] : 0.0f;
        d.w[tpos(d, (int)id, k)] = d.het ? side_pack((int)tk, ringa ? (ringa[(size_t)id * d.C + slot] & (TFX_MAX_ARCH - 1)) : 0) : tk;
      }
    }
    d.leadx[id] = row[ld].x;
    d.hb[id] = 0;
  }
}

__global__ void k_remi(const Dev d) {
  const long total = (long)d.E * d.I;
  for (long gid = (long)blockIdx.x * blockDim.x + threadIdx.x; gid < total;
       gid += (long)gridDim.x * blockDim.x) {
    const int env = (int)(gid / d.I);
    const int i = (int)(gid - (long)env * d.I);
    const int cur = d.obs[(size_t)env * d.obs_len + 2 * d.r + i];
    const bool pd = d.passed_dst[gid] != 0;
    float rw = 0.0f;
    for (int dir = 0; dir < 4; ++dir) {
      const int e = dir * d.I + i;
      const int phase_e = (dir < 2) ? 1 : 0;
      const bool green = phase_e != cur;
      int *wp = d.waiting + (size_t)env * d.r + e;
      const bool waiting = *wp > 0;
      if (waiting && !green && !pd) rw -= 0.5f;
      else if (pd && green && !waiting) rw += 0.5f;
      *wp = 0;
    }
    d.rewards[gid] = rw;
    d.passed_dst[gid] = 0;
  }
}

__global__ void k_cars_on_roads(const Dev d, int *out) {
  const long total = (long)d.E * d.R;
  for (long id = (long)blockIdx.x * blockDim.x + threadIdx.x; id < total;
       id += (long)gridDim.x * blockDim.x)
    out[id] = ring_count(d.leading[id], d.lastcar[id], d.C);
}

__global__ void k_done(const Dev d, uint8_t *out, int since_tick) {
  for (int env = blockIdx.x * blockDim.x + threadIdx.x; env < d.E; env += gridDim.x * blockDim.x)
    out[env] = d.done_tick[env] > since_tick ? 1 : 0;
}

__device__ __forceinline__ void philox4x32(unsigned c0, unsigned c1, unsigned c2, unsigned c3, unsigned k0,
                                           unsigned k1, unsigned out[4]) {
#pragma unroll
  for (int r = 0; r < 10; ++r) {
    const unsigned long long p0 = (unsigned long long)0xD2511F53u * c0;
    const unsigned long long p1 = (unsigned long long)0xCD9E8D57u * c2;
    const unsigned n0 = (unsigned)(p1 >> 32) ^ c1 ^ k0;
    const unsigned n1 = (unsigned)p1;
    const unsigned n2 = (unsigned)(p0 >> 32) ^ c3 ^ k1;
    const unsigned n3 = (unsigned)p0;
    c0 = n0; c1 = n1; c2 = n2; c3 = n3;
    k0 += 0x9E3779B9u;
    k1 += 0xBB67AE85u;
  }
  out[0] = c0; out[1] = c1; out[2] = c2; out[3] = c3;
}

struct PoissonDev {
  int *counts;
  int *gap_left;
  unsigned *draws;
  const unsigned *sid;
  const unsigned *cdf;
  int n_cdf;
  unsigned seed_lo, seed_hi;
  int regular, every, burst;
};

struct PoissonRows {
  uint8_t *rows;
  unsigned *seq;
  int S, n_arch;
};
constexpr unsigned TAG_ARCH = 0x41524348u;
constexpr unsigned TAG_EPISODE = 0x45504953u;
constexpr unsigned TAG_POOL = 0x504F4F4Cu;

__global__ void k_episode_begin(const Dev d, const EpDev ep) {
  const long total = (long)d.E * d.R;
  for (long id = (long)blockIdx.x * blockDim.x + threadIdx.x; id < total;
       id += (long)gridDim.x * blockDim.x) {
    const int env = (int)(id / d.R);
    const int e = (int)(id - (long)env * d.R);
    if (e == 0) ep.last[env] = (ep.max > 0 && ep.ep_len[env] + 1 == ep.max) ? 1 : 0;
    if (!ep.mark[env]) continue;
    int phase = 0;
    if (e < d.I) {
      unsigned u[4];
      philox4x32((unsigned)ep.ep_index[env], (unsigned)(env + d.env_off), TAG_EPISODE, (unsigned)e, ep.seed_lo,
                 ep.seed_hi, u);
      phase = (int)(u[0] & 1u);
    }
    reset_road(d, env, e, id, phase);
  }
}

__device__ __forceinline__ int episode_pool_slot(const EpDev &ep, const int env, const unsigned g, const int n_pool) {
  unsigned u[4];
  philox4x32((unsigned)ep.ep_index[env], g, TAG_POOL, 0u, ep.seed_lo, ep.seed_hi, u);
  return (int)(((unsigned long long)u[0] * (unsigned)n_pool) >> 32);
}

__device__ __forceinline__ void episode_add_reward(const EpDev &ep, const int env, const size_t gi, const float rw, const bool term) {
  float ret = ep.ep_return[gi] + rw;
  if (term || ep.last[env]) {
    ep.final_return[gi] = ret;
    ret = 0.0f;
  }
  ep.ep_return[gi] = ret;
}
__device__ __forceinline__ void episode_end_env(const EpDev &ep, const int env, const bool term) {
  const bool last = ep.last[env] != 0;
  int len = ep.ep_len[env] + 1;
  ep.trunc[env] = (!term && last) ? 1 : 0;
  if (term || last) {
    ep.final_len[env] = len;
    len = 0;
    ep.ep_index[env] += 1;
  }
  ep.ep_len[env] = len;
  ep.mark[env] = (term || last) ? 1 : 0;
}

template <bool ROWS>
__global__ __launch_bounds__(1024) void k_poisson(const Dev d, const PoissonDev ps, const int n_ticks, const PoissonRows pr) {
  extern __shared__ int s_hist[];
  int *s_first = s_hist + d.n_entry;
  unsigned *s_seq = (unsigned *)(s_first + 2);
  const int tid = threadIdx.x, nthr = blockDim.x;
  for (int env = blockIdx.x; env < d.E; env += gridDim.x) {
    const bool frozen = n_ticks == 1 && env_frozen(d, env, *d.tickA);
    int gap = ps.gap_left[env];
    unsigned c0 = ps.draws[env];
    const unsigned gid = ps.sid[env];
    unsigned u[4];
    if (ROWS)
      for (int j = tid; j < d.n_entry; j += nthr) s_seq[j] = pr.seq[(size_t)env * d.n_entry + j];
    auto gap_of = [&](unsigned draw) {
      philox4x32(draw, gid, 0x47415021u, 0u, ps.seed_lo, ps.seed_hi, u);
      int k = 0;
      while (k < ps.n_cdf - 1 && u[0] >= ps.cdf[k]) ++k;
      return k;
    };
    __syncthreads();
    for (int t = 0; t < n_ticks; ++t) {
      const unsigned c_tick = c0;
      for (int j = tid; j < d.n_entry; j += nthr) s_hist[j] = 0;
      __syncthreads();
      if (!frozen && ps.regular) {
        const bool due = ps.every == 0 || gap % ps.every == 0;
        ++gap;
        if (due) {
          for (int j = tid; j < ps.burst; j += nthr) {
            philox4x32(1u + 2u * (c0 + (unsigned)j), gid, 0x524F4144u, 0u, ps.seed_lo, ps.seed_hi, u);
            atomicAdd(&s_hist[(int)(((unsigned long long)u[0] * (unsigned)d.n_entry) >> 32)], 1);
          }
          c0 += (unsigned)ps.burst;
        }
      } else if (!frozen) {
        if (gap < 0) gap = gap_of(0u);
        if (gap > 0) {
          --gap;
        } else {
          for (int guard = 0; guard < 4096; ++guard) {
            if (tid == 0) { s_first[0] = 0x7fffffff; }
            __syncthreads();
            const unsigned c = c0 + (unsigned)tid;
            const int g = gap_of(2u + 2u * c);
            if (g > 0) atomicMin(&s_first[0], tid);
            __syncthreads();
            const int first = s_first[0];
            const int f = first < nthr ? first : nthr - 1;
            if (tid <= f) {
              philox4x32(1u + 2u * c, gid, 0x524F4144u, 0u, ps.seed_lo, ps.seed_hi, u);
              atomicAdd(&s_hist[(int)(((unsigned long long)u[0] * (unsigned)d.n_entry) >> 32)], 1);
            }
            if (tid == f) s_first[1] = g;
            c0 += (unsigned)(f + 1);
            __syncthreads();
            if (first < nthr) {
              gap = s_first[1] - 1;
              break;
            }
          }
        }
      }
      __syncthreads();
      if (ROWS && c0 != c_tick) {
        const int S = pr.S;
        const int dq = nthr / S, dr = nthr - dq * S;
        int ej = tid / S, j = tid - ej * S;
        uint8_t *rows = pr.rows + ((size_t)t * d.E + env) * d.n_entry * (size_t)S;
        while (ej < d.n_entry) {
          if (j < s_hist[ej]) {
            philox4x32(s_seq[ej] + (unsigned)j, gid, TAG_ARCH, (unsigned)ej, ps.seed_lo, ps.seed_hi, u);
            rows[(size_t)ej * S + j] = (uint8_t)(((unsigned long long)u[0] * (unsigned)pr.n_arch) >> 32);
          }
          j += dr;
          ej += dq;
          if (j >= S) { j -= S; ++ej; }
        }
        __syncthreads();
      }
      int *row = ps.counts + ((size_t)t * d.E + env) * d.n_entry;
      for (int j = tid; j < d.n_entry; j += nthr) {
        row[j] = s_hist[j];
        if (ROWS) s_seq[j] += (unsigned)s_hist[j];
      }
      __syncthreads();
    }
    if (tid == 0 && !frozen) {
      ps.gap_left[env] = gap;
      ps.draws[env] = c0;
    }
    if (ROWS && !frozen)
      for (int j = tid; j < d.n_entry; j += nthr) pr.seq[(size_t)env * d.n_entry + j] = s_seq[j];
  }
}

__global__ void k_greedy(const Dev d, int *action, int spacing) {
  const int tick = *d.tickA;
  if (tick % spacing != 0) return;
  const long total = (long)d.E * d.I;
  for (long g = (long)blockIdx.x * blockDim.x + threadIdx.x; g < total; g += (long)gridDim.x * blockDim.x) {
    const int env = (int)(g / d.I);
    action[g] = greedy_decide(d, env, (int)(g - (long)env * d.I));
  }
}

__global__ void k_agent_begin(const Dev d, int *first) { *first = *d.tickA; }

__global__ void k_clock_copy(const int *tickA, const int *tickB, int *clock2) {
  clock2[0] = *tickA;
  clock2[1] = *tickB;
}

__global__ void k_agent_tail(const Dev d, const int remi, float *aobs, float *areward, uint8_t *adone, const int *first,
                             const EpDev ep) {
  const int alen = 2 * d.r + d.I;
  const long n_int = (long)d.E * d.I, total = (long)d.E * alen;
  const int f = *first;
  for (long g = (long)blockIdx.x * blockDim.x + threadIdx.x; g < total; g += (long)gridDim.x * blockDim.x) {
    if (g < n_int) {
      float rw;
      if (remi) {
        const int env = (int)(g / d.I);
        const int i = (int)(g - (long)env * d.I);
        const int cur = d.obs[(size_t)env * d.obs_len + 2 * d.r + i];
        const bool pd = d.passed_dst[g] != 0;
        rw = 0.0f;
        for (int dir = 0; dir < 4; ++dir) {
          const bool green = ((dir < 2) ? 1 : 0) != cur;
          int *wp = d.waiting + (size_t)env * d.r + dir * d.I + i;
          const bool waiting = *wp > 0;
          if (waiting && !green && !pd) rw -= 0.5f;
          else if (pd && green && !waiting) rw += 0.5f;
          *wp = 0;
        }
        d.rewards[g] = rw;
        d.passed_dst[g] = 0;
      } else {
        rw = d.rewards[g];
      }
      if (areward) areward[g] = rw;
      if (ep.on) {
        const int env = (int)(g / d.I);
        episode_add_reward(ep, env, (size_t)g, rw, d.done_tick[env] > f);
      }
    }
    if (adone && g < d.E) adone[g] = d.done_tick[g] > f ? 1 : 0;
    if (ep.on && g < d.E) episode_end_env(ep, (int)g, d.done_tick[g] > f);
    if (aobs) {
      const int env = (int)(g / alen);
      const int k = (int)(g - (long)env * alen);
      const int *ob = d.obs + (size_t)env * d.obs_len;
      float v;
      if (k < 2 * d.r) {
        v = (float)ob[k];
      } else {
        const int i = k - 2 * d.r;
        v = (float)((double)ob[2 * d.r + d.I + i] / 100.0 * (double)(2 * ob[2 * d.r + i] - 1));
      }
      aobs[g] = v;
    }
  }
}

__global__ void k_div_selftest(float c, float rc, float lo, float hi, unsigned long long *mismatches) {
  const unsigned lo_b = __float_as_uint(lo), hi_b = __float_as_uint(hi);
  const unsigned long long n = (unsigned long long)(hi_b - lo_b) + 1ull;
  unsigned long long bad = 0;
  for (unsigned long long i = (unsigned long long)blockIdx.x * blockDim.x + threadIdx.x; i < 2 * n + 2;
       i += (unsigned long long)gridDim.x * blockDim.x) {
    unsigned bits;
    if (i < n) bits = lo_b + (unsigned)i;
    else if (i < 2 * n) bits = (lo_b + (unsigned)(i - n)) | 0x80000000u;
    else bits = (i == 2 * n) ? 0u : 0x80000000u;
    const float a = __uint_as_float(bits);
    const float want = a / c;
    const float got = div_const(a, c, rc);
    const bool same = (__float_as_uint(want) == __float_as_uint(got)) || (want == 0.0f && got == 0.0f);
    bad += same ? 0 : 1;
  }
  if (bad) atomicAdd(mismatches, bad);
}

}
```

### traffic-env_amd/csrc/tfx_move_tt.hpp

```cpp
#pragma once
#include <type_traits>

#include "tfx_common.hpp"
#include "tfx_move_t.hpp"

namespace tfx {

#ifndef TT_P
#define TT_P 4
#endif
#ifndef TT_WAVES
#define TT_WAVES 7
#endif
#ifndef TT_WAVES_AGENT
#define TT_WAVES_AGENT 6
#endif
#ifndef TT_WAVES_W
#define TT_WAVES_W 5
#endif
#ifndef TT_WAVES_TAIL
#define TT_WAVES_TAIL TT_WAVES
#endif
#define TT_ATTR_N(W, N) __attribute__((amdgpu_waves_per_eu((W) ? TT_WAVES_W : (N), (W) ? TT_WAVES_W : (N))))
#define TT_ATTR(W, AGENT) TT_ATTR_N(W, (AGENT) ? TT_WAVES_AGENT : TT_WAVES)
template <bool TWO, bool AGENT, bool W, bool HET, bool CREC = false, bool RSW = false>
__device__ __forceinline__ int move_tt_tile(const Dev &d, const long tile, const int env, const int lane, const int tick,
                                            const int tick_sp, const int tidx, const bool two, const float *s_arch,
                                            const bool skip = false) {
  constexpr int P = TT_P;
  const int C = d.C;
  const int e_slot = d.slot_road[(int)(tile - (long)env * d.G) * 64 + lane];
  const bool valid = e_slot >= 0;
  const int e = valid ? e_slot : 0;
  const int id = env * d.R + e;
  const int hb0 = (valid && !RSW) ? d.hb[id] : 0;
  const bool run = valid && !skip && !(AGENT && env_frozen(d, env, tick));
  const RoadPrep p = prep_road<RSW>(d, id, env, e, tick, tick_sp, tidx, run, run);
  const int hb = run ? (RSW ? p.hb : hb0) : 0;
  if (!RSW && hb) d.hb[id] = 0;
  const int n_old = run ? p.n_old : 0;
  const int n_sp = run ? p.n_tot - p.n_old : 0;

  char *const tb = reinterpret_cast<char *>(d.xv + ((size_t)tile * d.trows) * 64);
  char *const ox = reinterpret_cast<char *>(d.outb + ((size_t)tile * KP) * 64);
  const unsigned lo = (unsigned)lane * 8u;
  const unsigned ro = lo + (unsigned)hb * 512u;
  auto row_at = [&](char *base, unsigned k, unsigned off) {
    return reinterpret_cast<float2 *>(base + (size_t)(k * 512u + off));
  };
  float *wcol = W ? d.w + ((size_t)tile * d.trows) * 64 + lane : nullptr;
  float *owcol = W ? d.outw + ((size_t)tile * KP) * 64 + lane : nullptr;

  int kmax = n_old;
#pragma unroll
  for (int off = 32; off > 0; off >>= 1) {
    const int o = __shfl_xor(kmax, off, 64);
    kmax = o > kmax ? o : kmax;
  }
  kmax = __builtin_amdgcn_readfirstlane(kmax);

  float xprev = p.xL, vprev = 0.0f, llv = 0.0f;
  float y1x = 0.0f, y1v = 0.0f, y2x = 0.0f, y2v = 0.0f;
  float y1w = 0.0f;
  float y1l = 0.0f, y2l = 0.0f;
  int last_a = 0;
  int kpop = 0, n_wait = 0, n_det2 = 0;
  bool open = true, far = false;
  bool pend = false, pend_int = false;
  unsigned wo = lo;
  int kq1 = 0x7fffffff;
  float tail_x = 0.0f, tail_z = 0.0f;
  const int kq = (p.ld > p.lc) ? C - 1 - p.ld : 0x7fffffff;

  auto ld2 = [&](const float2 *ptr) {
    const f2v t = __builtin_nontemporal_load(reinterpret_cast<const f2v *>(ptr));
    return make_float2(t.x, t.y);
  };
  auto st2 = [&](float2 *ptr, float a, float b) {
    f2v t;
    t.x = a;
    t.y = b;
    __builtin_nontemporal_store(t, reinterpret_cast<f2v *>(ptr));
  };
  auto step = [&](int k, float x, float v, float sw, auto last) {
    constexpr bool LAST = decltype(last)::value;
    float xn = 0.0f, vn = 0.0f, zx = 0.0f, zv = 0.0f;
    const bool bad = !HET && ((!LAST && !idm_fast_domain(v)) || (TWO && two && !idm_fast_domain(y1v)));
    const bool off_domain = !HET && __builtin_amdgcn_ballot_w64(bad) != 0ull;
    float my_l = d.car_l;
    if (HET) {
      if (!LAST) {
        last_a = side_arch(sw);
        const float *me = s_arch + last_a * ARCH_W;
        idm_step_het(d, me, x, v, xprev, vprev, llv, xn, vn);
        my_l = me[AR_L];
      }
      if (TWO) idm_step_het(d, s_arch + side_arch(y1w) * ARCH_W, y1x, y1v, y2x, y2v, y2l, zx, zv);
    } else if (d.fastdiv && !off_domain) {
      if (!LAST) idm_step_fast(d, x, v, xprev, vprev, llv, xn, vn);
      if (TWO) idm_step_fast(d, y1x, y1v, y2x, y2v, d.car_l, zx, zv);
    } else {
      if (!LAST) idm_step(d, x, v, xprev, vprev, llv, xn, vn);
      if (TWO) idm_step(d, y1x, y1v, y2x, y2v, d.car_l, zx, zv);
    }
    if (TWO && two && pend) {
      st2(row_at(tb, 0, wo), pend_int ? zx : y1x, pend_int ? zv : y1v);
      if (W) wcol[(wo - lo) >> 3] = y1w;
      wo += 512u;
      if (pend_int) {
        const float wq1 = (k - 1 >= kq1) ? zx : zv;
        n_wait += (wq1 < d.thresh) ? 1 : 0;
        n_det2 += (zx > d.near_end) ? 0x10000 : 0;
        if (LAST) tail_z = zx;
      }
    }
    if (LAST) return;
    xprev = x;
    vprev = v;
    llv = my_l;
    const bool was_open = open;
    const bool pop = open && (xn > d.length);
    open = pop;
    if (pop) {
      if (kpop < KP) {
        *row_at(ox, 0, lo + (unsigned)kpop * 512u) = make_float2(xn, vn);
        if (W) owcol[(size_t)kpop * 64] = sw;
      } else {
        st2(row_at(tb, (unsigned)k, lo), xn, vn);
        if (W) wcol[(size_t)k * 64] = sw;
        wo = lo + (unsigned)(k + 1) * 512u;
      }
      far = far || ((xn - d.length) > d.length);
    } else if (TWO && two) {
      pend = true;
      pend_int = !was_open;
      if (was_open) kq1 = C - 1 - ring_adv(p.ld, kpop, C) + kpop;
    } else {
      st2(row_at(tb, 0, wo), xn, vn);
      if (W) wcol[(wo - lo) >> 3] = sw;
      wo += 512u;
    }
    kpop += pop ? 1 : 0;
    const float wq = (k >= kq) ? xn : vn;
    n_wait += (wq < d.thresh) ? 1 : 0;
    n_det2 += (xn > d.near_end) ? 1 : 0;
    if (!TWO) tail_x = xn;
    y2x = y1x;
    y2v = y1v;
    y1x = xn;
    y1v = vn;
    if (W) y1w = sw;
    if (HET) {
      y2l = y1l;
      y1l = my_l;
    }
  };

  float2 pf[P];
  float pfw[P];
  const float *wcolr = wcol + (size_t)hb * 64;
#pragma unroll
  for (int u = 0; u < P; ++u) {
    pf[u] = (u < n_old) ? ld2(row_at(tb, (unsigned)u, ro)) : make_float2(0.0f, 0.0f);
    pfw[u] = (W && u < n_old) ? wcolr[(size_t)u * 64] : 0.0f;
  }
  for (int k0 = 0; k0 < kmax; k0 += P) {
#pragma unroll
    for (int u = 0; u < P; ++u) {
      const int k = k0 + u;
      if (k < kmax) {
        const float2 cur = pf[u];
        const float curw = pfw[u];
        if (k + P < kmax) {
          pf[u] = (k + P < n_old) ? ld2(row_at(tb, (unsigned)(k + P), ro)) : make_float2(0.0f, 0.0f);
          pfw[u] = (W && k + P < n_old) ? wcolr[(size_t)(k + P) * 64] : 0.0f;
        }
        if (k < n_old) step(k, cur.x, cur.y, curw, std::false_type{});
      }
    }
  }
  if (__builtin_amdgcn_ballot_w64(n_sp > 0) != 0ull) {
    int smax = n_sp;
#pragma unroll
    for (int off = 32; off > 0; off >>= 1) {
      const int o = __shfl_xor(smax, off, 64);
      smax = o > smax ? o : smax;
    }
    smax = __builtin_amdgcn_readfirstlane(smax);
    if (HET) {
      int lcq = ring_adv(p.ld, n_old, C);
      float tx = d.tailx[id];
      int ta = d.taila[id];
      const int ej = d.entry_idx[e];
      const uint8_t *rows = (d.spawn_arch && d.spawn_mode == TFX_SPAWN_COUNTS && ej >= 0)
                                ? d.spawn_arch + (size_t)tidx * d.spawn_arch_stride +
                                      ((size_t)env * d.n_entry + ej) * d.spawn_arch_S
                                : nullptr;
      for (int s = 0; s < smax; ++s)
        if (s < n_sp) {
          const int row = (rows && s < d.spawn_arch_S) ? (rows[s] & (TFX_MAX_ARCH - 1)) : 0;
          const float start = (lcq != p.ld) ? (tx - s_arch[ta * ARCH_W + AR_L]) - s_arch[ta * ARCH_W + AR_S0] : INFINITY;
          const float xs = (start < 0.0f) ? start : 0.0f;
          step(n_old + s, xs, s_arch[row * ARCH_W + AR_V], side_pack(tick, row), std::false_type{});
          lcq = wrap1(lcq + 1, C);
          tx = xs;
          ta = row;
        }
    } else {
      for (int s = 0; s < smax; ++s)
        if (s < n_sp) step(n_old + s, spawned_x(d, p.xs0, s), d.car_v, (float)tick, std::false_type{});
    }
  }
  if (TWO && two && __builtin_amdgcn_ballot_w64(pend) != 0ull) {
    if (pend) step(p.n_tot, 0.0f, 0.0f, 0.0f, std::true_type{});
  }

  if (run) {
    const int n_tot = p.n_tot;
    const int n_det = n_det2 & 0xffff, n_det1 = n_det2 >> 16;
    if (e < d.r) {
      int *ob = d.obs + (size_t)env * d.obs_len;
      if (n_tot > 0 && !two) {
        d.waiting[(size_t)env * d.r + e] += n_wait;
        ob[d.r + e] = n_det;
      }
      if (AGENT && !two) ob[e] = (tidx > 0) ? ob[e] + kpop : kpop;
      else if (!two) ob[e] = kpop;
      if (kpop > 0) d.passed_dst[(size_t)env * d.I + e % d.I] = 1;
    }
    if (TWO) tail_x = y1x;
    if (TWO && CREC) {
      d.crec[id] = make_int2(crec_pack<HET>(kpop, n_tot, p.ld, p.lc, HET ? last_a : 0, kpop > KP, p.ovf_sp > 0), __float_as_int(tail_x));
      if (p.ovf_sp > 0) d.ovf_cnt[id] = p.ovf_sp;
    } else {
      d.rec[id] = make_int4(rec_pack(kpop, p.ld, C), rec_y(p.ovf_sp, kpop > KP), __float_as_int(tail_x),
                            n_tot | (HET ? last_a << 16 : 0));
    }
    if (two) {
      d.rec2f[id] = make_float2(y1v, tail_z);
      d.rec2c[id] = rec2c_pack(n_wait, n_det1, n_det, n_tot > 0);
    }
    if (far || kpop > KP) d.env_flag[env] = tick + 1;
    if (!two) d.leadx[id] = p.xL;
    return n_tot;
  }
  return 0;
}

template <bool TWO, bool AGENT = false, bool W = false, bool HET = false, bool CREC = false, bool RSW = false>
__global__ __launch_bounds__(256) TT_ATTR(W, AGENT) void k_move_tt(const Dev d, const int tidx, const int only_risky) {
  static_assert(!CREC || TWO, "only a two-tick pass is followed by k_tail");
  static_assert(!RSW || (CREC && !AGENT && !HET), "road state words: between the pairs of a plain tfx_step call");
  static_assert(!HET || W, "heterogeneous cars carry their table row in the side word");
  __shared__ float s_arch[HET ? TFX_MAX_ARCH * ARCH_W : 1];
  if (HET) load_arch(d, s_arch);
  const int lane = threadIdx.x & 63;
  const int wv = __builtin_amdgcn_readfirstlane(threadIdx.x >> 6);
  const int tick = *d.tickA;
  const long tiles = (long)d.E * d.G;
  const long nw = (long)gridDim.x * 4;
  const int tick_sp = (d.spawn_mode == TFX_SPAWN_PERIODIC) ? tick % d.spawn_period : 0;

  if (AGENT && only_risky && risk_any_word(d, tidx) != tick) return;

  unsigned long long my_updates = 0;

  for (long tile = (long)blockIdx.x * 4 + wv; tile < tiles; tile += nw) {
    const int env = (int)(tile / d.G);
    if (AGENT && only_risky && risk_word(d, env, tidx) != tick) continue;
    const bool sorted_out = AGENT && TWO && risk_word(d, env, tidx) == tick + 1;
    const bool two = TWO && (CREC || !sorted_out);
    if (AGENT && TWO && !two && lane == 0) risk_any_word(d, tidx) = tick + 1;
    my_updates += (unsigned long long)move_tt_tile<TWO, AGENT, W, HET, CREC, RSW>(d, tile, env, lane, tick, tick_sp, tidx, two, s_arch,
                                                                            CREC && sorted_out);
  }

  for (int off = 32; off > 0; off >>= 1) my_updates += __shfl_down(my_updates, off);
  if (lane == 0 && my_updates) veh_add(d.veh, my_updates);
  if (blockIdx.x == 0 && threadIdx.x == 0) *d.tickB = tick;
}

__device__ __forceinline__ bool risk_lane(const Dev &d, long tile, int env, int lane, int tick, int tick_sp, int tidx) {
  const int C = d.C;
  const int e = d.slot_road[(int)(tile - (long)env * d.G) * 64 + lane];
  if (e < 0) return false;
  const float half_ar2 = (0.5f * (d.risk_a * d.rate)) * d.rate;
  const int id = env * d.R + e;
  const int n = ring_count(d.leading[id], d.lastcar[id], C);
  const int ej = d.entry_idx[e];
  const int c_sp = ej >= 0 ? spawn_count(d, env, e, ej, tick_sp, tidx) : 0;
  bool risky = n + c_sp > C - 2;
  const float2 *col = d.xv + ((size_t)tile * d.trows) * 64 + lane + (size_t)d.hb[id] * 64;
  int pops = 0;
  const int n_look = (d.riskhint && d.riskhint[id] == 0) ? 0 : n;
  for (int j = 0; j <= KP && j < n_look; ++j) {
    const float2 c = col[(size_t)j * 64];
    const float reach = c.x + __builtin_fmaxf(d.rate * c.y + half_ar2, 0.0f);
    if (!(reach > d.length)) break;
    ++pops;
    if ((reach - d.length) > d.length) risky = true;
  }
  if (pops > KP) risky = true;
  const int nx = d.nexts[e];
  if (pops > 0 && nx >= 0) {
    const int idn = env * d.R + nx;
    if (ring_count(d.leading[idn], d.lastcar[idn], C) + pops > C - 2) risky = true;
  }
  return risky;
}

__global__ __launch_bounds__(256) void k_risk(const Dev d, const int tidx) {
  const int lane = threadIdx.x & 63;
  const int wv = __builtin_amdgcn_readfirstlane(threadIdx.x >> 6);
  const int tick = *d.tickA;
  const long tiles = (long)d.E * d.G;
  const long nw = (long)gridDim.x * 4;
  const int tick_sp = (d.spawn_mode == TFX_SPAWN_PERIODIC) ? tick % d.spawn_period : 0;
  for (long tile = (long)blockIdx.x * 4 + wv; tile < tiles; tile += nw) {
    const int env = (int)(tile / d.G);
    if (env_frozen(d, env, tick)) continue;
    if (risk_lane(d, tile, env, lane, tick, tick_sp, tidx)) {
      risk_word(d, env, tidx) = tick + 1;
      risk_any_word(d, tidx) = tick + 1;
    }
  }
}

template <bool AGENT, bool W = false, bool HET = false>
__device__ __forceinline__ int edge_tile(const Dev &d, long tile, int env, int lane, int tick, int tick_sp, int tidx,
                                         const float *arch = nullptr, const bool full_out = true) {
  const int C = d.C;
  if (AGENT && (risk_word(d, env, tidx) == tick || env_frozen(d, env, tick))) return 0;
  const int e = d.slot_road[(int)(tile - (long)env * d.G) * 64 + lane];
  if (e < 0) return 0;
  const int id = env * d.R + e;
  const int4 rc = d.rec[id];
  const int r2c = d.rec2c[id];
  const float2 r2f = d.rec2f[id];
  const RoadPrep p = prep_road(d, id, env, e, tick, tick_sp, tidx, true, true);
  const int m0 = rec_ntot(rc.w) - rec_kpop(rc.x);
  const int n_old = p.n_old, n_tot = p.n_tot;

  float2 *col = d.xv + ((size_t)tile * d.trows) * 64 + lane;
  float2 *ocol = d.outb + ((size_t)tile * KP) * 64 + lane;
  float *wcol = W ? d.w + ((size_t)tile * d.trows) * 64 + lane : nullptr;
  float *owcol = W ? d.outw + ((size_t)tile * KP) * 64 + lane : nullptr;

  int kpop = 0, n_wait = r2c & 1023, n_det = (r2c >> 10) & 511;
  bool open = true, far = false;
  const int kq = C - 1 - p.ld;
  float lx = p.xL, lv = 0.0f, ll = 0.0f;
  float tail_x = 0.0f;
  float hx = 0.0f, hv = 0.0f;
  int last_a = HET ? rec_taila(rc.w) : 0;
  auto car = [&](int i, float x, float v, bool fresh, float sw = 0.0f) {
    float zx, zv;
    if (HET) {
      if (!fresh) sw = wcol[(size_t)i * 64];
      last_a = side_arch(sw);
      const float *me = arch + last_a * ARCH_W;
      idm_step_het(d, me, x, v, lx, lv, ll, zx, zv);
      ll = me[AR_L];
    } else {
      if (W && fresh) sw = (float)tick;
      idm_step(d, x, v, lx, lv, ll, zx, zv);
      ll = d.car_l;
    }
    lx = x;
    lv = v;
    if (AGENT && i == 0) {
      hx = zx;
      hv = zv;
    }
    const bool pop = open && (zx > d.length);
    open = pop;
    if (pop && kpop < KP) {
      ocol[(size_t)kpop * 64] = make_float2(zx, zv);
      if (W) owcol[(size_t)kpop * 64] = fresh ? sw : wcol[(size_t)i * 64];
    } else {
      col[(size_t)i * 64] = make_float2(zx, zv);
      if (W && fresh) wcol[(size_t)i * 64] = sw;
    }
    if (pop) far = far || ((zx - d.length) > d.length);
    kpop += pop ? 1 : 0;
    const float wq = (i >= kq) ? zx : zv;
    n_wait += (wq < d.thresh) ? 1 : 0;
    n_det += (zx > d.near_end) ? 1 : 0;
    tail_x = zx;
  };
  if (m0 > 0) {
    const float2 head = col[0];
    car(0, head.x, head.y, false);
    for (int i = 1; i < m0 && open; ++i) {
      const float2 z = col[(size_t)i * 64];
      if (z.x > d.length) {
        if (kpop < KP) {
          ocol[(size_t)kpop * 64] = z;
          if (W) owcol[(size_t)kpop * 64] = wcol[(size_t)i * 64];
        }
        far = far || ((z.x - d.length) > d.length);
        ++kpop;
      } else {
        open = false;
      }
    }
    if (m0 >= 2) {
      lx = __int_as_float(rc.z);
      lv = r2f.x;
      tail_x = r2f.y;
      if (HET) {
        last_a = rec_taila(rc.w);
        ll = arch[last_a * ARCH_W + AR_L];
      }
    }
  }
  for (int i = m0; i < n_old; ++i) {
    const float2 c = col[(size_t)i * 64];
    car(i, c.x, c.y, false);
  }
  if (HET) {
    if (n_tot > n_old) {
      int lcq = ring_adv(p.ld, n_old, C);
      float tx = d.tailx[id];
      int ta = d.taila[id];
      const int ej = d.entry_idx[e];
      const uint8_t *rows = (d.spawn_arch && d.spawn_mode == TFX_SPAWN_COUNTS && ej >= 0)
                                ? d.spawn_arch + (size_t)tidx * d.spawn_arch_stride +
                                      ((size_t)env * d.n_entry + ej) * d.spawn_arch_S
                                : nullptr;
      for (int s = 0; s < n_tot - n_old; ++s) {
        const int row = (rows && s < d.spawn_arch_S) ? (rows[s] & (TFX_MAX_ARCH - 1)) : 0;
        const float start = (lcq != p.ld) ? (tx - arch[ta * ARCH_W + AR_L]) - arch[ta * ARCH_W + AR_S0] : INFINITY;
        const float xs = (start < 0.0f) ? start : 0.0f;
        car(n_old + s, xs, arch[row * ARCH_W + AR_V], true, side_pack(tick, row));
        lcq = wrap1(lcq + 1, C);
        tx = xs;
        ta = row;
      }
    }
  } else {
    for (int s = 0; s < n_tot - n_old; ++s) car(n_old + s, spawned_x(d, p.xs0, s), d.car_v, true);
  }

  const bool unc = kpop > KP;
  if (e < d.r) {
    int *ob = d.obs + (size_t)env * d.obs_len;
    if (n_wait != 0) d.waiting[(size_t)env * d.r + e] += n_wait;
    if (n_tot > 0) ob[d.r + e] = n_det;
    else if ((r2c >> 28) & 1) ob[d.r + e] = (r2c >> 19) & 511;
    if (AGENT) ob[e] = (tidx > 1 ? ob[e] : 0) + rec_kpop(rc.x) + kpop;
    else if (full_out) ob[e] = kpop;
    if (kpop > 0) d.passed_dst[(size_t)env * d.I + e % d.I] = 1;
  }
  if (!unc && kpop) d.hb[id] = (uint8_t)kpop;
  d.rec[id] = make_int4(rec_pack(kpop, p.ld, C), rec_y(p.ovf_sp, unc),
                        __float_as_int(tail_x), n_tot | (HET ? last_a << 16 : 0));
  if (far || unc) d.env_flag[env] = tick + 1;
  if (full_out || AGENT) d.leadx[id] = p.xL;
  if (AGENT && d.riskhint) {
    const float half_ar2 = (0.5f * (d.risk_a * d.rate)) * d.rate;
    const bool check = n_tot == 0 || kpop > 0 || (hx + __builtin_fmaxf(d.rate * hv + half_ar2, 0.0f)) > d.length;
    d.riskhint[id] = check ? 1 : 0;
  }
  return n_tot;
}

template <bool AGENT, bool W = false, bool HET = false>
__global__ __launch_bounds__(256) void k_edge(const Dev d, const int tidx) {
  __shared__ float s_arch[HET ? TFX_MAX_ARCH * ARCH_W : 1];
  if (HET) load_arch(d, s_arch);
  const int lane = threadIdx.x & 63;
  const int wv = __builtin_amdgcn_readfirstlane(threadIdx.x >> 6);
  const int tick = *d.tickA;
  const long tiles = (long)d.E * d.G;
  const long nw = (long)gridDim.x * 4;
  const int tick_sp = (d.spawn_mode == TFX_SPAWN_PERIODIC) ? tick % d.spawn_period : 0;

  unsigned long long my_updates = 0;
  for (long tile = (long)blockIdx.x * 4 + wv; tile < tiles; tile += nw)
    my_updates += (unsigned long long)edge_tile<AGENT, W, HET>(d, tile, (int)(tile / d.G), lane, tick, tick_sp, tidx, s_arch);

  for (int off = 32; off > 0; off >>= 1) my_updates += __shfl_down(my_updates, off);
  if (lane == 0 && my_updates) veh_add(d.veh, my_updates);
  if (blockIdx.x == 0 && threadIdx.x == 0) *d.tickB = tick;
}

}
```

### traffic-env_amd/csrc/tfx_sequence.hpp

```cpp
#pragma once
#include "tfx_clone.hpp"
#include "tfx_launch.hpp"

namespace {

int launch_pool_restart(tfx_handle h, hipStream_t st) {
  const tfx_handle pool = h->pool;
  CloneOpt o{};
  o.d_ep = h->ep;
  if (h->d.greedy_act && pool->d.greedy_act) {
    o.d_greedy = h->d.greedy_act;
    o.s_greedy = pool->d.greedy_act;
  }
  hipLaunchKernelGGL(k_clone<true>, dim3((unsigned)tile_grid(h)), dim3(256), 0, st, h->d, pool->d, (const int *)nullptr, o);
  HIPCHK(hipGetLastError());
  return TFX_OK;
}

int ensure_split(tfx_handle h, hipStream_t caller) {
  int lo = 0, hi = 0, cp = 0;
  HIPCHK(hipDeviceGetStreamPriorityRange(&lo, &hi));
  if (hipStreamGetPriority(caller, &cp) != hipSuccess) cp = 0;
  const int want = (cp == hi) ? lo : hi;
  if (h->split_stream && h->split_prio == want) return TFX_OK;
  if (h->split_stream) {
    HIPCHK(hipStreamSynchronize(h->split_stream));
    HIPCHK(hipStreamDestroy(h->split_stream));
    h->split_stream = nullptr;
  }
  HIPCHK(hipStreamCreateWithPriority(&h->split_stream, hipStreamNonBlocking, want));
  h->split_prio = want;
  if (h->split_fork) return TFX_OK;
  HIPCHK(hipEventCreateWithFlags(&h->split_fork, hipEventDisableTiming));
  HIPCHK(hipEventCreateWithFlags(&h->split_join, hipEventDisableTiming));
  HIPCHK(hipEventCreateWithFlags(&h->split_stagger, hipEventDisableTiming));
  return TFX_OK;
}

struct SeqGuard {
  tfx_handle h;
  Dev keep;
  hipStream_t user = nullptr;
  bool forked = false;
  explicit SeqGuard(tfx_handle hh) : h(hh), keep(hh->d) {}
  int fork(hipStream_t st) {
    user = st;
    HIPCHK(hipEventRecord(h->split_fork, st));
    HIPCHK(hipStreamWaitEvent(h->split_stream, h->split_fork, 0));
    forked = true;
    return TFX_OK;
  }
  int join() {
    if (!forked) return TFX_OK;
    forked = false;
    HIPCHK(hipEventRecord(h->split_join, h->split_stream));
    HIPCHK(hipStreamWaitEvent(user, h->split_join, 0));
    return TFX_OK;
  }
  ~SeqGuard() {
    h->d = keep;
    h->split_half = -1;
    h->split_first = false;
    if (forked) {
      const std::string first = g_err;
      (void)join();
      g_err = first;
    }
  }
};

struct TickTimer {
  tfx_handle h;
  hipEvent_t *e = nullptr;
  explicit TickTimer(tfx_handle hh) : h(hh) {}
  int begin(hipStream_t st) {
    if (!h->prof || h->ev_used >= h->ev_ticks) return TFX_OK;
    e = &h->ev[(size_t)h->ev_used * 3];
    HIPCHK(hipEventRecord(e[0], st));
    return TFX_OK;
  }
  int mid(hipStream_t st) {
    if (e) HIPCHK(hipEventRecord(e[1], st));
    return TFX_OK;
  }
  int end(hipStream_t st, int weight) {
    if (!e) return TFX_OK;
    HIPCHK(hipEventRecord(e[2], st));
    h->ev_weight[h->ev_used] = weight;
    ++h->ev_used;
    return TFX_OK;
  }
};

int pair(tfx_handle h, int t, int n_ticks, hipStream_t st, bool agent) {
  const bool tail = tail_usable(h);
  TickTimer timer(h);
  if (int rc = launch_inputs(h, st)) return rc;
  if (agent && !(tail && t > 0)) {
    if (int rc = launch_risk(h, t, st)) return rc;
  }
  if (!agent) {
    if (int rc = timer.begin(st)) return rc;
  }
  if (int rc = launch_move_tt(h, true, agent, t, st, 0, tail, agent ? false : t > 0)) return rc;
  if (int rc = timer.mid(st)) return rc;
  if (tail) {
    const int flags = (t + 2 >= n_ticks ? TAIL_LAST : 0) |
                      (agent ? (t + 3 < n_ticks ? TAIL_RISK_NEXT : 0) : (t + 3 >= n_ticks ? TAIL_SYNC : 0));
    if (int rc = launch_tail(h, t, st, agent, flags)) return rc;
    if (!agent) h->tail_ticks += 2;
  } else {
    if (int rc = launch_advance(h, t, st)) return rc;
    if (int rc = launch_inputs(h, st)) return rc;
    if (int rc = launch_edge(h, agent, t + 1, st)) return rc;
    if (agent) {
      if (int rc = launch_move_tt(h, false, true, t + 1, st, 1)) return rc;
    }
    if (int rc = launch_advance(h, t + 1, st)) return rc;
  }
  if (int rc = timer.end(st, 2)) return rc;
  h->pair_ticks += 2;
  return TFX_OK;
}

int single(tfx_handle h, int t, hipStream_t st, bool agent) {
  TickTimer timer(h);
  if (int rc = launch_inputs(h, st)) return rc;
  if (!agent) {
    if (int rc = timer.begin(st)) return rc;
  }
  if (int rc = (pairs_usable(h) && !single_tick_ts(h)) ? launch_move_tt(h, false, agent, t, st) : launch_move(h, t, st)) return rc;
  if (int rc = timer.mid(st)) return rc;
  if (int rc = launch_advance(h, t, st)) return rc;
  return timer.end(st, 1);
}

int run_ticks(tfx_handle h, int n_ticks, hipStream_t st, bool agent, bool split) {
  SeqGuard guard(h);
  const Dev whole = h->d;
  Dev halves[2] = {whole, whole};
  if (split) {
    hipLaunchKernelGGL(k_clock_copy, dim3(1), dim3(1), 0, st, whole.tickA, whole.tickB, h->misc->clock2);
    HIPCHK(hipGetLastError());
    if (int rc = guard.fork(st)) return rc;
    const int n0 = whole.E / 2;
    halves[0] = sub_dev(whole, 0, n0, nullptr);
    halves[1] = sub_dev(whole, n0, whole.E - n0, h->misc->clock2);
  }
  const long long pair0 = h->pair_ticks, tail0 = h->tail_ticks;
  const int turn = split ? 2 : n_ticks;
  int rc = TFX_OK;
  for (int t0 = 0; t0 < n_ticks && rc == TFX_OK; t0 += turn) {
    for (int half = 0; half < (split ? 2 : 1) && rc == TFX_OK; ++half) {
      if (split) {
        h->d = halves[half];
        h->split_half = half;
        h->split_first = t0 == 0;
      }
      const hipStream_t hs = half == 0 ? st : h->split_stream;
      const int t_hi = t0 + turn < n_ticks ? t0 + turn : n_ticks;
      int t = t0;
      if (pairs_usable(h))
        for (; t + 1 < t_hi && rc == TFX_OK; t += 2) rc = pair(h, t, n_ticks, hs, agent);
      for (; t < t_hi && rc == TFX_OK; ++t) rc = single(h, t, hs, agent);
    }
  }
  if (!split) return rc;
  h->d = whole;
  h->split_half = -1;
  h->pair_ticks = pair0 + (h->pair_ticks - pair0) / 2;
  h->tail_ticks = tail0 + (h->tail_ticks - tail0) / 2;
  if (rc != TFX_OK) return rc;
  h->split_ticks += n_ticks;
  return guard.join();
}

int agent_sequence(tfx_handle h, int n_ticks, int remi, float *aobs, float *areward, uint8_t *adone,
                   hipStream_t st, bool split) {
  Dev &d = h->d;
  SeqGuard guard(h);
  if (h->ep.on) {
    TFX_INJECT(h);
    if (h->pool) {
      if (int rc = launch_pool_restart(h, st)) return rc;
    } else {
      hipLaunchKernelGGL(k_episode_begin, dim3(grid_for(h, (long)d.E * d.R)), dim3(256), 0, st, d, h->ep);
      HIPCHK(hipGetLastError());
    }
  }
  if (h->stream.upfront()) {
    if (int rc = launch_stream(h, n_ticks, st)) return rc;
  }
  if (res_usable(h, n_ticks)) {
    d.agent_mode = 1;
    d.accum_rewards = remi ? 0 : 1;
    const int rc = launch_res(h, n_ticks, st, 1, remi, aobs, areward, adone);
    if (rc == TFX_OK) h->fused_ticks += n_ticks;
    return rc;
  }
  hipLaunchKernelGGL(k_agent_begin, dim3(1), dim3(1), 0, st, d, const_cast<int *>(d.agent_first));
  HIPCHK(hipGetLastError());
  if (int rc = launch_greedy(h, st)) return rc;
  d.agent_mode = 1;
  d.accum_rewards = remi ? 0 : 1;
  if (int rc = run_ticks(h, n_ticks, st, true, split)) return rc;
  d.agent_mode = guard.keep.agent_mode;
  d.accum_rewards = guard.keep.accum_rewards;
  if (remi || aobs || areward || adone || h->ep.on) {
    hipLaunchKernelGGL(k_agent_tail, dim3(grid_for(h, (long)d.E * (2 * d.r + d.I))), dim3(256), 0, st, d, remi, aobs,
                       areward, adone, d.agent_first, h->ep);
    HIPCHK(hipGetLastError());
  }
  return TFX_OK;
}

}
```

### traffic-env_amd/csrc/tfx_tail.hpp

```cpp
#pragma once
#include "tfx_advance.hpp"
#include "tfx_common.hpp"
#include "tfx_move_tt.hpp"

namespace tfx {

enum { TAIL_RISK_NEXT = 1, TAIL_LAST = 2, TAIL_SYNC = 4 };

inline size_t tail_lds_bytes(int R, int I, bool het) {
  return (size_t)R * (sizeof(int4) + 4 * sizeof(int) + (het ? sizeof(int) : 0)) + (size_t)2 * I * sizeof(int) + 2 * (((size_t)R + 15) & ~(size_t)15);
}

template <bool GREEDY = false, bool AGENT = false, bool W = false, bool HET = false>
__global__ __launch_bounds__(256) TT_ATTR_N(W, AGENT ? TT_WAVES_AGENT : TT_WAVES_TAIL) void k_tail(const Dev d, const int tidx, const int flags) {
  static_assert(!HET || W, "heterogeneous cars carry their table row in the side word");
  extern __shared__ int4 s_dyn[];
  __shared__ float s_arch[HET ? TFX_MAX_ARCH * ARCH_W : 1];
  if (HET) load_arch(d, s_arch);
  const int lane = threadIdx.x & 63;
  const int wv = __builtin_amdgcn_readfirstlane(threadIdx.x >> 6);
  const int nwv = blockDim.x >> 6;
  const int tick = *d.tickB;
  const int per_env = d.I + (d.R - d.r);
  const int sp0 = (d.spawn_mode == TFX_SPAWN_PERIODIC) ? (tick + 1) % d.spawn_period : 0;
  const int R = d.R;
  const int risk_next = flags & TAIL_RISK_NEXT;
  const bool full_out = (flags & TAIL_LAST) != 0;
  int4 *const s_rec = s_dyn;
  int *const s_ld = reinterpret_cast<int *>(s_rec + R);
  int *const s_lc = s_ld + R;
  float *const s_tx = reinterpret_cast<float *>(s_lc + R);
  int *const s_ta = reinterpret_cast<int *>(s_tx + R);
  int *const s_lt = s_ta + (HET ? R : 0);
  uint8_t *const s_hb = reinterpret_cast<uint8_t *>(s_lt + 2 * d.I);
  uint8_t *const s_hint = s_hb + ((R + 15) & ~15);
  float *const s_lx = reinterpret_cast<float *>(s_hint + ((R + 15) & ~15));

  unsigned long long my_updates = 0;
  for (int env = blockIdx.x; env < d.E; env += gridDim.x) {
    Dev dl = d;
    const size_t base = (size_t)env * R;
    const bool sorted_out = AGENT && risk_word(d, env, tidx) == tick + 1;
    const bool frozen0 = AGENT && env_frozen(d, env, tick);
    const bool packed = !HET && !sorted_out && !frozen0;
    {
      for (int e = threadIdx.x; e < R; e += blockDim.x) {
        const int2 c = d.crec[base + e];
        s_rec[e] = crec_expand<HET>(c, crec_ovf<HET>(c.x) ? d.ovf_cnt[base + e] : 0, d.C);
        if (packed) {
          s_ld[e] = (c.x >> 9) & 511;
          s_lc[e] = (c.x >> 18) & 511;
          s_hb[e] = 0;
        } else {
          s_ld[e] = d.leading[base + e];
          s_lc[e] = d.lastcar[base + e];
          s_tx[e] = d.tailx[base + e];
          s_hb[e] = d.hb[base + e];
        }
        if (HET) s_ta[e] = d.taila[base + e];
      }
      const int *lt = d.lights + (size_t)env * d.lights_stride;
      for (int i = threadIdx.x; i < 2 * d.I; i += blockDim.x) s_lt[i] = lt[i];
      dl.rec = s_rec - base;
      dl.leading = s_ld - base;
      dl.lastcar = s_lc - base;
      dl.tailx = s_tx - base;
      if (HET) dl.taila = s_ta - base;
      dl.hb = s_hb - base;
      if (AGENT) {
        dl.leadx = s_lx - base;
        dl.riskhint = sorted_out ? nullptr : s_hint - base;
      }
      dl.lights = s_lt;
      dl.lights_stride = 0;
      __syncthreads();
    }
    if (AGENT && sorted_out) {
      if (threadIdx.x == 0) atomicAdd(d.slow_pairs, 1ull);
      for (int u = 0; u < 2; ++u) {
        const int spu = (d.spawn_mode == TFX_SPAWN_PERIODIC) ? (tick + u) % d.spawn_period : 0;
        if (u) __syncthreads();
        for (int g = wv; g < d.G; g += nwv)
          my_updates += (unsigned long long)move_tt_tile<false, AGENT, W, HET>(dl, (long)env * d.G + g, env, lane, tick + u, spu, tidx + u, false, s_arch);
        __syncthreads();
        for (int s = threadIdx.x; s < per_env; s += blockDim.x) advance_item<true, HET, GREEDY, W>(dl, env, s, tick + u, tidx + u);
      }
    } else {
      for (int s = threadIdx.x; s < per_env; s += blockDim.x) advance_item<true, HET, GREEDY, W>(dl, env, s, tick, tidx);
      __syncthreads();
      for (int g = wv; g < d.G; g += nwv)
        my_updates += (unsigned long long)edge_tile<AGENT, W, HET>(dl, (long)env * d.G + g, env, lane, tick + 1, sp0, tidx + 1, s_arch, full_out);
      __syncthreads();
      for (int s = threadIdx.x; s < per_env; s += blockDim.x) advance_item<true, HET, GREEDY, W>(dl, env, s, tick + 1, tidx + 1);
    }
    if (AGENT && risk_next) {
      __syncthreads();
      const int t2 = tick + 2;
      if (!env_frozen(d, env, t2)) {
        const int sp2 = (d.spawn_mode == TFX_SPAWN_PERIODIC) ? t2 % d.spawn_period : 0;
        bool risky = false;
        for (int g = wv; g < d.G; g += nwv) risky = risk_lane(dl, (long)env * d.G + g, env, lane, t2, sp2, tidx + 2) || risky;
        if (__builtin_amdgcn_ballot_w64(risky) != 0ull && lane == 0) risk_word(d, env, tidx + 2) = t2 + 1;
      }
    }
    {
      __syncthreads();
      for (int e = threadIdx.x; e < R; e += blockDim.x) {
        if (AGENT || HET || (flags & TAIL_SYNC)) {
          d.hb[base + e] = s_hb[e];
          d.leading[base + e] = s_ld[e];
          d.lastcar[base + e] = s_lc[e];
        } else {
          d.rsw[base + e] = rsw_pack(s_ld[e], s_lc[e], s_hb[e]);
        }
        d.tailx[base + e] = s_tx[e];
        if (HET) d.taila[base + e] = s_ta[e];
      }
      int *lt = d.lights + (size_t)env * d.lights_stride;
      for (int i = threadIdx.x; i < 2 * d.I; i += blockDim.x) lt[i] = s_lt[i];
      if (AGENT && !frozen0 && (full_out || d.done_tick[env] > *d.agent_first))
        for (int e = threadIdx.x; e < R; e += blockDim.x) d.leadx[base + e] = s_lx[e];
      __syncthreads();
    }
  }

  for (int off = 32; off > 0; off >>= 1) my_updates += __shfl_down(my_updates, off);
  if (lane == 0 && my_updates) veh_add(d.veh, my_updates);
  if (blockIdx.x == 0 && threadIdx.x == 0) *d.tickA = tick + 2;
}

}
```

### traffic-env_amd/gym_traffic/_native.py

```python
import ctypes as C
import os

_HERE = os.path.dirname(os.path.abspath(__file__))
LIB_PATH = os.environ.get("TFX_LIB", os.path.join(os.path.dirname(_HERE), "lib", "libtfx_hip.so"))

MAX_ARCH = 64
ACTION_BUFFER, ACTION_BROADCAST, ACTION_CYCLE, ACTION_GREEDY = 0, 1, 2, 3
SPAWN_NONE, SPAWN_COUNTS, SPAWN_PERIODIC = 0, 1, 2
ABI_VERSION = 13
CLONE_STREAM, CLONE_EPISODE = 1, 2
MEASURE_ACCUMULATE = 1
CELLS_ACCUMULATE = 1
MAX_CELLS = 32
TRAVEL_ACCUMULATE = 1
MAX_TRIP_BINS = 32
FRAMES_ROADS_ONLY = 1
FOLLOW_ACCUMULATE = 1
FRAME_PX_MIN, FRAME_PX_MAX = 8, 256
DEMAND_MAX_PROFILES, DEMAND_MAX_SEGMENTS, DEMAND_MAX_CDF = 16, 64, 256


class TfxConfig(C.Structure):
    _fields_ = [("m", C.c_int32), ("n", C.c_int32), ("capacity", C.c_int32), ("n_envs", C.c_int32),
                ("planes", C.c_int32), ("length", C.c_float), ("rate", C.c_float),
                ("car_v", C.c_float), ("car_l", C.c_float), ("car_a", C.c_float),
                ("car_delta", C.c_float), ("car_v0", C.c_float), ("car_b", C.c_float),
                ("car_T", C.c_float), ("car_s0", C.c_float),
                ("yellow_ticks", C.c_int32), ("thresh", C.c_float), ("detect_dist", C.c_float),
                ("overflow_penalty", C.c_float), ("eps", C.c_float),
                ("learn_switch", C.c_int32), ("validate", C.c_int32), ("entry_spec", C.c_uint32),
                ("env_id_offset", C.c_int32), ("layout", C.c_int32),
                ("n_archetypes", C.c_int32), ("arch", (C.c_float * 8) * MAX_ARCH)]


class TfxBuffers(C.Structure):
    _fields_ = [("xv", C.c_void_p), ("w", C.c_void_p), ("leading", C.c_void_p), ("lastcar", C.c_void_p),
                ("obs", C.c_void_p), ("rewards", C.c_void_p), ("waiting", C.c_void_p),
                ("passed_dst", C.c_void_p), ("done_tick", C.c_void_p),
                ("trip_times", C.c_void_p), ("n_trips", C.c_void_p), ("trip_cap", C.c_int32)]


class TfxEpisodeBuffers(C.Structure):
    _fields_ = [("ep_return", C.c_void_p), ("ep_len", C.c_void_p), ("final_return", C.c_void_p),
                ("final_len", C.c_void_p), ("truncated", C.c_void_p), ("ep_index", C.c_void_p)]


class TfxMeasureBuffers(C.Structure):
    _fields_ = [("n_cars", C.c_void_p), ("n_halted", C.c_void_p), ("queue", C.c_void_p), ("speed_sum", C.c_void_p)]


class TfxCellBuffers(C.Structure):
    _fields_ = [("n_cars", C.c_void_p), ("speed_sum", C.c_void_p)]


class TfxAgeBuffers(C.Structure):
    _fields_ = [("n_cars", C.c_void_p), ("age_sum", C.c_void_p), ("age_max", C.c_void_p)]


class TfxTripStatBuffers(C.Structure):
    _fields_ = [("count", C.c_void_p), ("tick_sum", C.c_void_p), ("tick_max", C.c_void_p), ("lost", C.c_void_p),
                ("hist", C.c_void_p)]


class TfxFollowParams(C.Structure):
    _fields_ = [("x_from", C.c_float), ("platoon_gap", C.c_float), ("v_min", C.c_float), ("ttc_crit", C.c_float)]


class TfxFollowBuffers(C.Structure):
    _fields_ = [("n_cars", C.c_void_p), ("n_pairs", C.c_void_p), ("n_joined", C.c_void_p), ("n_overlap", C.c_void_p),
                ("gap_sum", C.c_void_p), ("gap_min", C.c_void_p), ("n_hw", C.c_void_p), ("hw_sum", C.c_void_p),
                ("n_conflict", C.c_void_p), ("ttc_min", C.c_void_p), ("drac_max", C.c_void_p)]


class TfxDemand(C.Structure):
    _fields_ = [("n_profiles", C.c_int32), ("n_segments", C.c_int32), ("seg_ticks", C.c_int32),
                ("tick_offset", C.c_int32), ("n_cdf", C.c_int32),
                ("count_cdf", C.c_void_p), ("road_cdf", C.c_void_p), ("profile_of_env", C.c_void_p),
                ("seed", C.c_uint64)]


class TfxError(RuntimeError):
    pass


_lib = None

_PROTOS = {
    "tfx_abi_version": (C.c_int, []),
    "tfx_last_error": (C.c_char_p, []),
    "tfx_create": (C.c_int, [C.POINTER(TfxConfig), C.POINTER(C.c_void_p)]),
    "tfx_destroy": (C.c_int, [C.c_void_p]),
    "tfx_dims": (C.c_int, [C.c_void_p] + [C.POINTER(C.c_int32)] * 4),
    "tfx_tables": (C.c_int, [C.c_void_p] + [C.c_void_p] * 4),
    "tfx_bind_buffers": (C.c_int, [C.c_void_p, C.POINTER(TfxBuffers)]),
    "tfx_reset": (C.c_int, [C.c_void_p, C.c_void_p, C.c_void_p]),
    "tfx_reset_envs": (C.c_int, [C.c_void_p, C.c_void_p, C.c_void_p, C.c_void_p]),
    "tfx_refresh": (C.c_int, [C.c_void_p, C.c_void_p]),
    "tfx_set_episodes": (C.c_int, [C.c_void_p, C.c_int32, C.c_int32, C.c_uint64, C.POINTER(TfxEpisodeBuffers)]),
    "tfx_set_episode_pool": (C.c_int, [C.c_void_p, C.c_void_p]),
    "tfx_set_actions": (C.c_int, [C.c_void_p, C.c_int32, C.c_void_p, C.c_int32, C.c_int32]),
    "tfx_set_spawns": (C.c_int, [C.c_void_p, C.c_int32, C.c_void_p, C.c_int32, C.c_int32]),
    "tfx_set_poisson": (C.c_int, [C.c_void_p, C.c_double, C.c_uint64, C.c_void_p, C.c_int32]),
    "tfx_set_regular": (C.c_int, [C.c_void_p, C.c_int32, C.c_int32, C.c_uint64]),
    "tfx_set_spawn_archetypes": (C.c_int, [C.c_void_p, C.c_void_p, C.c_int32, C.c_int32]),
    "tfx_set_demand": (C.c_int, [C.c_void_p, C.POINTER(TfxDemand)]),
    "tfx_demand_counts": (C.c_int, [C.c_void_p, C.c_int32, C.c_int32, C.c_void_p, C.c_void_p]),
    "tfx_set_demand_mixed": (C.c_int, [C.c_void_p, C.POINTER(TfxDemand), C.c_void_p, C.c_int32]),
    "tfx_demand_rows": (C.c_int, [C.c_void_p, C.c_int32, C.c_int32, C.c_void_p, C.c_void_p, C.c_void_p]),
    "tfx_demand_rows_per_road": (C.c_int, [C.c_void_p, C.POINTER(C.c_int32)]),
    "tfx_step": (C.c_int, [C.c_void_p, C.c_int32, C.c_void_p]),
    "tfx_move_cars": (C.c_int, [C.c_void_p, C.c_void_p]),
    "tfx_advance_finished_cars": (C.c_int, [C.c_void_p, C.c_void_p]),
    "tfx_agent_step": (C.c_int, [C.c_void_p, C.c_int32, C.c_int32, C.c_void_p, C.c_void_p, C.c_void_p, C.c_void_p]),
    "tfx_remi": (C.c_int, [C.c_void_p, C.c_void_p]),
    "tfx_cars_on_roads": (C.c_int, [C.c_void_p, C.c_void_p, C.c_void_p]),
    "tfx_done": (C.c_int, [C.c_void_p, C.c_void_p, C.c_int32, C.c_void_p]),
    "tfx_get_tick": (C.c_int, [C.c_void_p, C.POINTER(C.c_int32)]),
    "tfx_set_tick": (C.c_int, [C.c_void_p, C.c_int32]),
    "tfx_vehicle_updates": (C.c_int, [C.c_void_p, C.POINTER(C.c_uint64), C.c_void_p]),
    "tfx_reset_counters": (C.c_int, [C.c_void_p, C.c_void_p]),
    "tfx_profile": (C.c_int, [C.c_void_p, C.c_int32]),
    "tfx_profile_read": (C.c_int, [C.c_void_p, C.POINTER(C.c_double), C.POINTER(C.c_double), C.POINTER(C.c_int32)]),
    "tfx_xv_pairs": (C.c_int, [C.c_void_p, C.POINTER(C.c_int64)]),
    "tfx_export_ring": (C.c_int, [C.c_void_p, C.c_void_p, C.c_void_p, C.c_void_p, C.c_void_p]),
    "tfx_import_ring": (C.c_int, [C.c_void_p, C.c_void_p, C.c_void_p, C.c_void_p, C.c_void_p]),
    "tfx_fastdiv_status": (C.c_int, [C.c_void_p, C.POINTER(C.c_int32), C.POINTER(C.c_uint64)]),
    "tfx_launch_info": (C.c_int, [C.c_void_p] + [C.POINTER(C.c_int32)] * 3),
    "tfx_arrivals_replay": (C.c_int, [C.c_void_p, C.c_int32, C.c_int32, C.c_int32, C.c_double, C.c_int32, C.c_int32,
                                      C.c_int32, C.c_void_p, C.c_int32, C.c_void_p, C.c_void_p]),
    "tfx_arrivals_replay_rows": (C.c_int, [C.c_void_p, C.c_int32, C.c_int32, C.c_int32, C.c_double, C.c_int32,
                                           C.c_int32, C.c_int32, C.c_void_p, C.c_int32, C.c_void_p, C.c_void_p,
                                           C.c_int32, C.c_int32, C.c_void_p]),
    "tfx_fused_ticks": (C.c_int, [C.c_void_p, C.POINTER(C.c_int64), C.POINTER(C.c_int32)]),
    "tfx_pair_ticks": (C.c_int, [C.c_void_p, C.POINTER(C.c_int64)]),
    "tfx_tail_ticks": (C.c_int, [C.c_void_p, C.POINTER(C.c_int64)]),
    "tfx_slow_pairs": (C.c_int, [C.c_void_p, C.POINTER(C.c_uint64), C.c_void_p]),
    "tfx_split_ticks": (C.c_int, [C.c_void_p, C.POINTER(C.c_int64)]),
    "tfx_step_kernel": (C.c_char_p, [C.c_void_p]),
    "tfx_debug_fail_after": (C.c_int, [C.c_void_p, C.c_int32]),
    "tfx_clone_envs": (C.c_int, [C.c_void_p, C.c_void_p, C.c_void_p, C.c_int32, C.c_void_p]),
    "tfx_clone_skipped": (C.c_int, [C.c_void_p, C.POINTER(C.c_uint64), C.c_void_p]),
    "tfx_debug_head_rows": (C.c_int, [C.c_void_p, C.c_void_p, C.c_void_p]),
    "tfx_road_measures": (C.c_int, [C.c_void_p, C.c_float, C.c_float, C.POINTER(TfxMeasureBuffers), C.c_int32, C.c_void_p]),
    "tfx_measure_launch": (C.c_int, [C.c_void_p, C.POINTER(C.c_int32), C.POINTER(C.c_int32)]),
    "tfx_road_cells": (C.c_int, [C.c_void_p, C.POINTER(C.c_float), C.c_int32, C.POINTER(TfxCellBuffers), C.c_int32, C.c_void_p]),
    "tfx_cells_launch": (C.c_int, [C.c_void_p, C.c_int32, C.POINTER(C.c_int32), C.POINTER(C.c_int32)]),
    "tfx_car_ages": (C.c_int, [C.c_void_p, C.POINTER(TfxAgeBuffers), C.c_int32, C.c_void_p]),
    "tfx_ages_launch": (C.c_int, [C.c_void_p, C.POINTER(C.c_int32), C.POINTER(C.c_int32)]),
    "tfx_trip_stats": (C.c_int, [C.c_void_p, C.POINTER(C.c_int32), C.c_int32, C.c_void_p, C.POINTER(TfxTripStatBuffers),
                                 C.c_int32, C.c_void_p]),
    "tfx_frame_size": (C.c_int, [C.c_void_p, C.c_int32, C.POINTER(C.c_int32), C.POINTER(C.c_int32)]),
    "tfx_frames": (C.c_int, [C.c_void_p, C.c_void_p, C.c_int32, C.c_int32, C.c_void_p, C.c_int32, C.c_void_p]),
    "tfx_frames_launch": (C.c_int, [C.c_void_p, C.c_int32, C.c_int32, C.POINTER(C.c_int32), C.POINTER(C.c_int32)]),
    "tfx_road_following": (C.c_int, [C.c_void_p, C.POINTER(TfxFollowParams), C.POINTER(TfxFollowBuffers), C.c_int32,
                                     C.c_void_p]),
    "tfx_follow_launch": (C.c_int, [C.c_void_p, C.POINTER(C.c_int32), C.POINTER(C.c_int32)]),
}


def lib():
    global _lib
    if _lib is None:
        if not os.path.exists(LIB_PATH):
            raise TfxError("HIP library not found at %s - build it with `python -c 'import "
                           "__graft_entry__ as g; g.build()'` (or make -C traffic-env_amd/csrc). "
                           "There is no CPU fallback for the env step." % LIB_PATH)
        try:
            handle = C.CDLL(LIB_PATH)
        except OSError as exc:
            raise TfxError("cannot load %s: %s" % (LIB_PATH, exc))
        for name, (res, argtypes) in _PROTOS.items():
            fn = getattr(handle, name)
            fn.restype = res
            fn.argtypes = argtypes
        if handle.tfx_abi_version() != ABI_VERSION:
            raise TfxError("libtfx_hip.so ABI %d != binding ABI %d" % (handle.tfx_abi_version(), ABI_VERSION))
        _lib = handle
    return _lib


def check(rc):
    if rc != 0:
        raise TfxError("tfx error %d: %s" % (rc, lib().tfx_last_error().decode("utf-8", "replace")))
    return rc
```

Before: 540.8 billion vehicle-updates/s.

## Carry risk stamps across agent-step calls and fold greedy/clock into agent_begin

```diff
diff --git a/include/tfx.h b/include/tfx.h
--- a/include/tfx.h
+++ b/include/tfx.h
@@ -217,6 +217,7 @@
                        void *stream);
 int tfx_follow_launch(tfx_handle h, int32_t *grid, int32_t *waves);
 int tfx_debug_head_rows(tfx_handle h, uint8_t *out, void *stream);
+int tfx_debug_risk_stamps(tfx_handle h, int32_t set, int32_t *stamped);
 
 typedef struct tfx_arrival_stream {
   uint32_t mt[624];
diff --git a/traffic-env_amd/csrc/tfx_handle.hpp b/traffic-env_amd/csrc/tfx_handle.hpp
--- a/traffic-env_amd/csrc/tfx_handle.hpp
+++ b/traffic-env_amd/csrc/tfx_handle.hpp
@@ -135,7 +135,11 @@
   int device = 0;
   int measure_grid = 0;
   int grid_cap = 0;
+  bool risk_stamped = false;
+  bool risk_launch = false;
 };
+
+inline void stamps_clear(tfx_handle_s *h) { h->risk_stamped = false; }
 
 namespace {
 
@@ -206,4 +210,10 @@
   return TFX_OK;
 }
 
-}
+int check_mutator(tfx_handle h, bool need_bound) {
+  if (int rc = check_handle(h, need_bound)) return rc;
+  stamps_clear(h);
+  return TFX_OK;
+}
+
+}
diff --git a/traffic-env_amd/csrc/tfx_hip.hip b/traffic-env_amd/csrc/tfx_hip.hip
--- a/traffic-env_amd/csrc/tfx_hip.hip
+++ b/traffic-env_amd/csrc/tfx_hip.hip
@@ -99,9 +99,19 @@
     if (int rc = ensure_split(h, st)) return rc;
   }
   const bool capture = h->use_graph && !split;
-  auto body = [&](hipStream_t s) { return agent_sequence(h, n_ticks, remi, aobs, areward, adone, s, split); };
-  if (!capture) return body(st);
-  return run_captured(h, h->captured[SEQ_AGENT], graph_key(h, n_ticks, remi, aobs, areward, adone), st, body);
+  const int stamps = (h->risk_stamped && !h->risk_launch ? STAMPS_HELD : 0) | (stamps_left(h, n_ticks) ? STAMPS_LEAVE : 0);
+  stamps_clear(h);
+  auto body = [&](hipStream_t s) { return agent_sequence(h, n_ticks, remi, aobs, areward, adone, s, split, stamps); };
+  int rc;
+  if (!capture) {
+    rc = body(st);
+  } else {
+    std::string key = graph_key(h, n_ticks, remi, aobs, areward, adone);
+    key_put(key, stamps);
+    rc = run_captured(h, h->captured[SEQ_AGENT], key, st, body);
+  }
+  if (rc == TFX_OK && (stamps & STAMPS_LEAVE)) h->risk_stamped = true;
+  return rc;
 }
 
 namespace {
@@ -187,6 +197,7 @@
 void install_stream(tfx_handle h, ArrivalStream &&s) {
   Dev &d = h->d;
   ++h->input_gen;
+  stamps_clear(h);
   drop_stream(h);
   h->stream = std::move(s);
   const ArrivalStream &a = h->stream;
@@ -221,7 +232,7 @@
     if (const int c = bad_cdf_row(dm->count_cdf + (size_t)ks * n_cdf, n_cdf))
       return fail(TFX_EINVAL, c < n_cdf ? "demand: count_cdf row (%d, %d) decreases at %d" : "demand: count_cdf row (%d, %d) does not end in 0xFFFFFFFF",
                   ks / S, ks % S, c);
-  if (int rc = check_handle(h, false)) return rc;
+  if (int rc = check_mutator(h, false)) return rc;
   Dev &d = h->d;
   if (h->het && !mixed)
     return fail(TFX_EINVAL, "demand: heterogeneous handles (tfx_config.n_archetypes) are not supported - rule 4 draws no archetype rows: "
@@ -355,6 +366,7 @@
   if (const char *gv = getenv("TFX_GRID_CAP")) h->grid_cap = atoi(gv) > 0 ? atoi(gv) : 0;
   if (const char *pc = getenv("TFX_MOVE_BLOCKS_PER_CU")) h->move_blocks_per_cu = atoi(pc);
   if (const char *sv = getenv("TFX_STAGGER")) h->stagger = atoi(sv) != 0;
+  if (const char *rv = getenv("TFX_RISK_LAUNCH")) h->risk_launch = atoi(rv) != 0;
   int dev = 0;
   hipDeviceProp_t prop;
   if (hipGetDevice(&dev) == hipSuccess) h->device = dev;
@@ -528,7 +540,7 @@
 }
 
 int tfx_bind_buffers(tfx_handle h, const tfx_buffers *b) {
-  if (int rc = check_handle(h, false)) return rc;
+  if (int rc = check_mutator(h, false)) return rc;
   if (!b) return fail(TFX_EINVAL, "null buffers");
   if (!b->xv || !b->leading || !b->lastcar || !b->obs || !b->rewards || !b->waiting ||
       !b->passed_dst || !b->done_tick)
@@ -550,7 +562,7 @@
 }
 
 int tfx_reset(tfx_handle h, const int32_t *phase_init, void *stream) {
-  if (int rc = check_handle(h, true)) return rc;
+  if (int rc = check_mutator(h, true)) return rc;
   if (!phase_init) return fail(TFX_EINVAL, "phase_init is required");
   hipStream_t st = (hipStream_t)stream;
   HIPCHK(hipMemsetAsync(h->d.tickA, 0, sizeof(int), st));
@@ -562,7 +574,7 @@
 }
 
 int tfx_reset_envs(tfx_handle h, const int32_t *phase_init, const uint8_t *mask, void *stream) {
-  if (int rc = check_handle(h, true)) return rc;
+  if (int rc = check_mutator(h, true)) return rc;
   if (!phase_init || !mask) return fail(TFX_EINVAL, "phase_init and mask are required");
   hipLaunchKernelGGL(k_reset, dim3(grid_for(h, (long)h->d.E * h->d.R)), dim3(256), 0, (hipStream_t)stream,
                      h->d, phase_init, mask, h->ep);
@@ -577,7 +589,7 @@
     if (!b->ep_return || !b->ep_len || !b->final_return || !b->final_len || !b->truncated || !b->ep_index)
       return fail(TFX_EINVAL, "ep_return, ep_len, final_return, final_len, truncated and ep_index are required");
   }
-  if (int rc = check_handle(h, true)) return rc;
+  if (int rc = check_mutator(h, true)) return rc;
   EpDev &ep = h->ep;
   HIPCHK(hipDeviceSynchronize());
   HIPCHK(hipMemset(ep.mark, 0, 2 * (size_t)h->d.E));
@@ -598,7 +610,7 @@
 }
 
 int tfx_refresh(tfx_handle h, void *stream) {
-  if (int rc = check_handle(h, true)) return rc;
+  if (int rc = check_mutator(h, true)) return rc;
   hipLaunchKernelGGL(k_refresh, dim3(grid_for(h, (long)h->d.E * h->d.R)), dim3(256), 0,
                      (hipStream_t)stream, h->d);
   HIPCHK(hipGetLastError());
@@ -606,7 +618,7 @@
 }
 
 int tfx_set_actions(tfx_handle h, int32_t mode, const int32_t *dev, int32_t period, int32_t per_tick) {
-  if (int rc = check_handle(h, false)) return rc;
+  if (int rc = check_mutator(h, false)) return rc;
   Dev &d = h->d;
   ++h->input_gen;
   h->greedy = false;
@@ -644,7 +656,7 @@
 }
 
 int tfx_set_spawns(tfx_handle h, int32_t mode, const int32_t *dev, int32_t period, int32_t per_tick) {
-  if (int rc = check_handle(h, false)) return rc;
+  if (int rc = check_mutator(h, false)) return rc;
   Dev &d = h->d;
   ++h->input_gen;
   drop_stream(h);
@@ -664,7 +676,7 @@
 }
 
 int tfx_set_spawn_archetypes(tfx_handle h, const uint8_t *dev, int32_t per_road, int32_t per_tick) {
-  if (int rc = check_handle(h, false)) return rc;
+  if (int rc = check_mutator(h, false)) return rc;
   if (!h->het) return fail(TFX_ESTATE, "the handle has a single archetype");
   if (dev && per_road < 1) return fail(TFX_EINVAL, "per_road must be >= 1");
   Dev &d = h->d;
@@ -676,7 +688,7 @@
 }
 
 int tfx_set_poisson(tfx_handle h, double cars_per_tick, uint64_t seed, const uint32_t *cdf, int32_t n_cdf) {
-  if (int rc = check_handle(h, false)) return rc;
+  if (int rc = check_mutator(h, false)) return rc;
   if (!(cars_per_tick > 0.0)) return fail(TFX_EINVAL, "cars_per_tick must be > 0");
   if (!cdf || n_cdf < 1 || n_cdf > 65536) return fail(TFX_EINVAL, "gap table missing or too long");
   Dev &d = h->d;
@@ -691,7 +703,7 @@
 }
 
 int tfx_set_regular(tfx_handle h, int32_t every, int32_t burst, uint64_t seed) {
-  if (int rc = check_handle(h, false)) return rc;
+  if (int rc = check_mutator(h, false)) return rc;
   if (every < 0 || burst < 1) return fail(TFX_EINVAL, "every must be >= 0 and burst >= 1");
   Dev &d = h->d;
   if (d.n_entry < 1) return fail(TFX_EINVAL, "no entry roads");
@@ -740,7 +752,7 @@
 }
 
 int tfx_step(tfx_handle h, int32_t n_ticks, void *stream) {
-  if (int rc = check_handle(h, true)) return rc;
+  if (int rc = check_mutator(h, true)) return rc;
   if (n_ticks < 0) return fail(TFX_EINVAL, "n_ticks < 0");
   hipStream_t st = (hipStream_t)stream;
   if (n_ticks > 0 && res_usable(h, n_ticks)) {
@@ -764,7 +776,7 @@
 }
 
 int tfx_move_cars(tfx_handle h, void *stream) {
-  if (int rc = check_handle(h, true)) return rc;
+  if (int rc = check_mutator(h, true)) return rc;
   if (int rc = size_grids(h, false, 1)) return rc;
   if (int rc = launch_greedy(h, (hipStream_t)stream)) return rc;
   if (int rc = h->stream.upfront() ? launch_stream(h, 1, (hipStream_t)stream) : launch_inputs(h, (hipStream_t)stream)) return rc;
@@ -772,7 +784,7 @@
 }
 
 int tfx_advance_finished_cars(tfx_handle h, void *stream) {
-  if (int rc = check_handle(h, true)) return rc;
+  if (int rc = check_mutator(h, true)) return rc;
   if (int rc = size_grids(h, false, 1)) return rc;
   return launch_advance(h, 0, (hipStream_t)stream);
 }
@@ -812,7 +824,7 @@
 }
 
 int tfx_set_tick(tfx_handle h, int32_t tick) {
-  if (int rc = check_handle(h, false)) return rc;
+  if (int rc = check_mutator(h, false)) return rc;
   HIPCHK(hipDeviceSynchronize());
   HIPCHK(hipMemcpy(h->d.tickA, &tick, sizeof(int), hipMemcpyHostToDevice));
   HIPCHK(hipMemcpy(h->d.tickB, &tick, sizeof(int), hipMemcpyHostToDevice));
@@ -840,7 +852,7 @@
 }
 
 int tfx_profile(tfx_handle h, int32_t max_ticks) {
-  if (int rc = check_handle(h, false)) return rc;
+  if (int rc = check_mutator(h, false)) return rc;
   for (hipEvent_t e : h->ev) (void)hipEventDestroy(e);
   h->ev.clear();
   h->ev_ticks = 0;
@@ -892,7 +904,7 @@
 }
 
 int tfx_import_ring(tfx_handle h, const float *ring_xv, const float *ring_w, const uint8_t *ring_a, void *stream) {
-  if (int rc = check_handle(h, true)) return rc;
+  if (int rc = check_mutator(h, true)) return rc;
   if (h->d.layout != 1) return fail(TFX_ESTATE, "the handle already uses the ring layout");
   if (!ring_xv) return fail(TFX_EINVAL, "ring_xv is null");
   hipLaunchKernelGGL(k_import_ring, dim3(grid_for(h, (long)h->d.E * h->d.R)), dim3(256), 0,
@@ -1007,7 +1019,7 @@
 int tfx_clone_envs(tfx_handle dst, tfx_handle src, const int32_t *src_of_env, int32_t flags, void *stream) {
   if (flags & ~(TFX_CLONE_STREAM | TFX_CLONE_EPISODE)) return fail(TFX_EINVAL, "unknown clone flags 0x%x", flags);
   if (!src_of_env) return fail(TFX_EINVAL, "src_of_env is null");
-  if (int rc = check_handle(dst, true)) return rc;
+  if (int rc = check_mutator(dst, true)) return rc;
   if (int rc = check_handle(src, true)) return rc;
   if (dst != src) {
     if (int rc = same_world(dst, src, "clone")) return rc;
@@ -1045,7 +1057,7 @@
 }
 
 int tfx_set_episode_pool(tfx_handle h, tfx_handle pool) {
-  if (int rc = check_handle(h, false)) return rc;
+  if (int rc = check_mutator(h, false)) return rc;
   if (pool == h) return fail(TFX_EINVAL, "episode pool: a handle cannot be its own pool");
   if (int rc = check_handle(h, true)) return rc;
   if (pool) {
@@ -1270,6 +1282,13 @@
   return TFX_OK;
 }
 
+int tfx_debug_risk_stamps(tfx_handle h, int32_t set, int32_t *stamped) {
+  if (int rc = check_handle(h, false)) return rc;
+  if (set >= 0) h->risk_stamped = set != 0;
+  if (stamped) *stamped = h->risk_stamped ? 1 : 0;
+  return TFX_OK;
+}
+
 int tfx_debug_fail_after(tfx_handle h, int32_t n_launches) {
   if (int rc = check_handle(h, false)) return rc;
   h->fail_after = n_launches > 0 ? n_launches : 0;
diff --git a/traffic-env_amd/csrc/tfx_misc.hpp b/traffic-env_amd/csrc/tfx_misc.hpp
--- a/traffic-env_amd/csrc/tfx_misc.hpp
+++ b/traffic-env_amd/csrc/tfx_misc.hpp
@@ -335,7 +335,25 @@
   }
 }
 
-__global__ void k_agent_begin(const Dev d, int *first) { *first = *d.tickA; }
+__global__ void k_agent_begin(const Dev d, int *first, int *action, int spacing, int *clock2, int restamp) {
+  const int tick = *d.tickA;
+  if (blockIdx.x == 0 && threadIdx.x == 0) {
+    *first = tick;
+    if (clock2) {
+      clock2[0] = tick;
+      clock2[1] = *d.tickB;
+    }
+  }
+  if (restamp)
+    for (int env = blockIdx.x * blockDim.x + threadIdx.x; env < d.E; env += gridDim.x * blockDim.x)
+      if (d.env_risk[env] == tick + 1) d.env_risk[env] = 0;
+  if (!action || tick % spacing != 0) return;
+  const long total = (long)d.E * d.I;
+  for (long g = (long)blockIdx.x * blockDim.x + threadIdx.x; g < total; g += (long)gridDim.x * blockDim.x) {
+    const int env = (int)(g / d.I);
+    action[g] = greedy_decide(d, env, (int)(g - (long)env * d.I));
+  }
+}
 
 __global__ void k_clock_copy(const int *tickA, const int *tickB, int *clock2) {
   clock2[0] = *tickA;
diff --git a/traffic-env_amd/csrc/tfx_move_tt.hpp b/traffic-env_amd/csrc/tfx_move_tt.hpp
--- a/traffic-env_amd/csrc/tfx_move_tt.hpp
+++ b/traffic-env_amd/csrc/tfx_move_tt.hpp
@@ -280,19 +280,10 @@
   if (blockIdx.x == 0 && threadIdx.x == 0) *d.tickB = tick;
 }
 
-__device__ __forceinline__ bool risk_lane(const Dev &d, long tile, int env, int lane, int tick, int tick_sp, int tidx) {
+__device__ __forceinline__ bool risk_heads(const Dev &d, const float2 *col, int n_look, int env, int e, bool risky) {
   const int C = d.C;
-  const int e = d.slot_road[(int)(tile - (long)env * d.G) * 64 + lane];
-  if (e < 0) return false;
   const float half_ar2 = (0.5f * (d.risk_a * d.rate)) * d.rate;
-  const int id = env * d.R + e;
-  const int n = ring_count(d.leading[id], d.lastcar[id], C);
-  const int ej = d.entry_idx[e];
-  const int c_sp = ej >= 0 ? spawn_count(d, env, e, ej, tick_sp, tidx) : 0;
-  bool risky = n + c_sp > C - 2;
-  const float2 *col = d.xv + ((size_t)tile * d.trows) * 64 + lane + (size_t)d.hb[id] * 64;
   int pops = 0;
-  const int n_look = (d.riskhint && d.riskhint[id] == 0) ? 0 : n;
   for (int j = 0; j <= KP && j < n_look; ++j) {
     const float2 c = col[(size_t)j * 64];
     const float reach = c.x + __builtin_fmaxf(d.rate * c.y + half_ar2, 0.0f);
@@ -307,6 +298,33 @@
     if (ring_count(d.leading[idn], d.lastcar[idn], C) + pops > C - 2) risky = true;
   }
   return risky;
+}
+
+__device__ __forceinline__ bool risk_road(const Dev &d, int env, int e, int tick, int tick_sp, int tidx) {
+  const int id = env * d.R + e;
+  const int n = ring_count(d.leading[id], d.lastcar[id], d.C);
+  const int ej = d.entry_idx[e];
+  const int c_sp = ej >= 0 ? spawn_count(d, env, e, ej, tick_sp, tidx) : 0;
+  const bool risky = n + c_sp > d.C - 2;
+  const int n_look = (d.riskhint && d.riskhint[id] == 0) ? 0 : n;
+  if (n_look == 0) return risky;
+  const int slot = d.road_slot[e];
+  const float2 *col = d.xv + (((size_t)env * d.G + (slot >> 6)) * d.trows) * 64 + (slot & 63) + (size_t)d.hb[id] * 64;
+  return risk_heads(d, col, n_look, env, e, risky);
+}
+
+__device__ __forceinline__ bool risk_lane(const Dev &d, long tile, int env, int lane, int tick, int tick_sp, int tidx) {
+  const int C = d.C;
+  const int e = d.slot_road[(int)(tile - (long)env * d.G) * 64 + lane];
+  if (e < 0) return false;
+  const int id = env * d.R + e;
+  const int n = ring_count(d.leading[id], d.lastcar[id], C);
+  const int ej = d.entry_idx[e];
+  const int c_sp = ej >= 0 ? spawn_count(d, env, e, ej, tick_sp, tidx) : 0;
+  const bool risky = n + c_sp > C - 2;
+  const float2 *col = d.xv + ((size_t)tile * d.trows) * 64 + lane + (size_t)d.hb[id] * 64;
+  const int n_look = (d.riskhint && d.riskhint[id] == 0) ? 0 : n;
+  return risk_heads(d, col, n_look, env, e, risky);
 }
 
 __global__ __launch_bounds__(256) void k_risk(const Dev d, const int tidx) {
diff --git a/traffic-env_amd/csrc/tfx_sequence.hpp b/traffic-env_amd/csrc/tfx_sequence.hpp
--- a/traffic-env_amd/csrc/tfx_sequence.hpp
+++ b/traffic-env_amd/csrc/tfx_sequence.hpp
@@ -92,11 +92,20 @@
   }
 };
 
-int pair(tfx_handle h, int t, int n_ticks, hipStream_t st, bool agent) {
+enum { STAMPS_HELD = 1, STAMPS_LEAVE = 2 };
+
+bool stamps_left(tfx_handle h, int n_ticks) {
+  const Dev &d = h->d;
+  if (h->risk_launch || res_usable(h, n_ticks) || !pairs_usable(h, n_ticks) || !tail_usable(h)) return false;
+  if ((n_ticks & 1) || h->ep.on || d.het || d.w || h->stream.drawn()) return false;
+  return d.spawn_mode == TFX_SPAWN_PERIODIC || d.spawn_mode == TFX_SPAWN_NONE;
+}
+
+int pair(tfx_handle h, int t, int n_ticks, hipStream_t st, bool agent, int stamps = 0) {
   const bool tail = tail_usable(h);
   TickTimer timer(h);
   if (int rc = launch_inputs(h, st)) return rc;
-  if (agent && !(tail && t > 0)) {
+  if (agent && !(tail && (t > 0 || (stamps & STAMPS_HELD)))) {
     if (int rc = launch_risk(h, t, st)) return rc;
   }
   if (!agent) {
@@ -106,7 +115,8 @@
   if (int rc = timer.mid(st)) return rc;
   if (tail) {
     const int flags = (t + 2 >= n_ticks ? TAIL_LAST : 0) |
-                      (agent ? (t + 3 < n_ticks ? TAIL_RISK_NEXT : 0) : (t + 3 >= n_ticks ? TAIL_SYNC : 0));
+                      (agent ? (t + 3 < n_ticks ? TAIL_RISK_NEXT : 0) : (t + 3 >= n_ticks ? TAIL_SYNC : 0)) |
+                      (agent && (stamps & STAMPS_LEAVE) && t + 2 == n_ticks ? TAIL_RISK_CALL : 0);
     if (int rc = launch_tail(h, t, st, agent, flags)) return rc;
     if (!agent) h->tail_ticks += 2;
   } else {
@@ -135,13 +145,15 @@
   return timer.end(st, 1);
 }
 
-int run_ticks(tfx_handle h, int n_ticks, hipStream_t st, bool agent, bool split) {
+int run_ticks(tfx_handle h, int n_ticks, hipStream_t st, bool agent, bool split, int stamps = 0) {
   SeqGuard guard(h);
   const Dev whole = h->d;
   Dev halves[2] = {whole, whole};
   if (split) {
-    hipLaunchKernelGGL(k_clock_copy, dim3(1), dim3(1), 0, st, whole.tickA, whole.tickB, h->misc->clock2);
-    HIPCHK(hipGetLastError());
+    if (!agent) {
+      hipLaunchKernelGGL(k_clock_copy, dim3(1), dim3(1), 0, st, whole.tickA, whole.tickB, h->misc->clock2);
+      HIPCHK(hipGetLastError());
+    }
     if (int rc = guard.fork(st)) return rc;
     const int n0 = whole.E / 2;
     halves[0] = sub_dev(whole, 0, n0, nullptr);
@@ -161,7 +173,7 @@
       const int t_hi = t0 + turn < n_ticks ? t0 + turn : n_ticks;
       int t = t0;
       if (pairs_usable(h))
-        for (; t + 1 < t_hi && rc == TFX_OK; t += 2) rc = pair(h, t, n_ticks, hs, agent);
+        for (; t + 1 < t_hi && rc == TFX_OK; t += 2) rc = pair(h, t, n_ticks, hs, agent, stamps);
       for (; t < t_hi && rc == TFX_OK; ++t) rc = single(h, t, hs, agent);
     }
   }
@@ -176,7 +188,7 @@
 }
 
 int agent_sequence(tfx_handle h, int n_ticks, int remi, float *aobs, float *areward, uint8_t *adone,
-                   hipStream_t st, bool split) {
+                   hipStream_t st, bool split, int stamps) {
   Dev &d = h->d;
   SeqGuard guard(h);
   if (h->ep.on) {
@@ -198,12 +210,13 @@
     if (rc == TFX_OK) h->fused_ticks += n_ticks;
     return rc;
   }
-  hipLaunchKernelGGL(k_agent_begin, dim3(1), dim3(1), 0, st, d, const_cast<int *>(d.agent_first));
+  hipLaunchKernelGGL(k_agent_begin, dim3(h->greedy ? grid_for(h, (long)d.E * d.I) : 1), dim3(256), 0, st, d,
+                     const_cast<int *>(d.agent_first), h->greedy ? h->dev_greedy : nullptr, h->greedy_spacing,
+                     split ? h->misc->clock2 : nullptr, (stamps & STAMPS_HELD) ? 0 : 1);
   HIPCHK(hipGetLastError());
-  if (int rc = launch_greedy(h, st)) return rc;
   d.agent_mode = 1;
   d.accum_rewards = remi ? 0 : 1;
-  if (int rc = run_ticks(h, n_ticks, st, true, split)) return rc;
+  if (int rc = run_ticks(h, n_ticks, st, true, split, stamps)) return rc;
   d.agent_mode = guard.keep.agent_mode;
   d.accum_rewards = guard.keep.accum_rewards;
   if (remi || aobs || areward || adone || h->ep.on) {
diff --git a/traffic-env_amd/csrc/tfx_tail.hpp b/traffic-env_amd/csrc/tfx_tail.hpp
--- a/traffic-env_amd/csrc/tfx_tail.hpp
+++ b/traffic-env_amd/csrc/tfx_tail.hpp
@@ -5,7 +5,7 @@
 
 namespace tfx {
 
-enum { TAIL_RISK_NEXT = 1, TAIL_LAST = 2, TAIL_SYNC = 4 };
+enum { TAIL_RISK_NEXT = 1, TAIL_LAST = 2, TAIL_SYNC = 4, TAIL_RISK_CALL = 8 };
 
 inline size_t tail_lds_bytes(int R, int I, bool het) {
   return (size_t)R * (sizeof(int4) + 4 * sizeof(int) + (het ? sizeof(int) : 0)) + (size_t)2 * I * sizeof(int) + 2 * (((size_t)R + 15) & ~(size_t)15);
@@ -25,6 +25,7 @@
   const int sp0 = (d.spawn_mode == TFX_SPAWN_PERIODIC) ? (tick + 1) % d.spawn_period : 0;
   const int R = d.R;
   const int risk_next = flags & TAIL_RISK_NEXT;
+  const int risk_call = flags & TAIL_RISK_CALL;
   const bool full_out = (flags & TAIL_LAST) != 0;
   int4 *const s_rec = s_dyn;
   int *const s_ld = reinterpret_cast<int *>(s_rec + R);
@@ -42,6 +43,10 @@
     const size_t base = (size_t)env * R;
     const bool sorted_out = AGENT && risk_word(d, env, tidx) == tick + 1;
     const bool frozen0 = AGENT && env_frozen(d, env, tick);
+    if (AGENT && (risk_next || risk_call) && threadIdx.x == 0) {
+      int &next = risk_word(d, env, risk_call ? 0 : tidx + 2);
+      if (next == tick + 3) next = 0;
+    }
     const bool packed = !HET && !sorted_out && !frozen0;
     {
       for (int e = threadIdx.x; e < R; e += blockDim.x) {
@@ -93,14 +98,17 @@
       __syncthreads();
       for (int s = threadIdx.x; s < per_env; s += blockDim.x) advance_item<true, HET, GREEDY, W>(dl, env, s, tick + 1, tidx + 1);
     }
-    if (AGENT && risk_next) {
+    if (AGENT && (risk_next || risk_call)) {
       __syncthreads();
       const int t2 = tick + 2;
-      if (!env_frozen(d, env, t2)) {
+      const bool stopped = env_frozen(d, env, t2);
+      if (risk_call || !stopped) {
+        if (stopped) dl.riskhint = nullptr;
         const int sp2 = (d.spawn_mode == TFX_SPAWN_PERIODIC) ? t2 % d.spawn_period : 0;
+        const int tnext = risk_call ? 0 : tidx + 2;
         bool risky = false;
-        for (int g = wv; g < d.G; g += nwv) risky = risk_lane(dl, (long)env * d.G + g, env, lane, t2, sp2, tidx + 2) || risky;
-        if (__builtin_amdgcn_ballot_w64(risky) != 0ull && lane == 0) risk_word(d, env, tidx + 2) = t2 + 1;
+        for (int e = threadIdx.x; e < R; e += blockDim.x) risky = risk_road(dl, env, e, t2, sp2, tnext) || risky;
+        if (__builtin_amdgcn_ballot_w64(risky) != 0ull && lane == 0) risk_word(d, env, tnext) = t2 + 1;
       }
     }
     {
diff --git a/traffic-env_amd/gym_traffic/_native.py b/traffic-env_amd/gym_traffic/_native.py
--- a/traffic-env_amd/gym_traffic/_native.py
+++ b/traffic-env_amd/gym_traffic/_native.py
@@ -141,6 +141,7 @@
     "tfx_clone_envs": (C.c_int, [C.c_void_p, C.c_void_p, C.c_void_p, C.c_int32, C.c_void_p]),
     "tfx_clone_skipped": (C.c_int, [C.c_void_p, C.POINTER(C.c_uint64), C.c_void_p]),
     "tfx_debug_head_rows": (C.c_int, [C.c_void_p, C.c_void_p, C.c_void_p]),
+    "tfx_debug_risk_stamps": (C.c_int, [C.c_void_p, C.c_int32, C.POINTER(C.c_int32)]),
     "tfx_road_measures": (C.c_int, [C.c_void_p, C.c_float, C.c_float, C.POINTER(TfxMeasureBuffers), C.c_int32, C.c_void_p]),
     "tfx_measure_launch": (C.c_int, [C.c_void_p, C.POINTER(C.c_int32), C.POINTER(C.c_int32)]),
     "tfx_road_cells": (C.c_int, [C.c_void_p, C.POINTER(C.c_float), C.c_int32, C.POINTER(TfxCellBuffers), C.c_int32, C.c_void_p]),
```

Result: no change. 540.8 billion vehicle-updates/s, median of 2 (-0.0%).
